# AlexeyAB/yolo2_light

Hardware: NVIDIA H100
Metric: images/sec (higher is better)
Workload: dtype bf16

## Files before the change

### yolo2_light_b200/csrc/yb_conv_tc.cu

```cuda
#include <cuda.h>
#include <cuda_bf16.h>
#include <cuda_runtime.h>

#include <algorithm>
#include <climits>
#include <cstdlib>
#include <cstring>
#include <memory>
#include <string>
#include <type_traits>
#include <vector>

#include "yb_conv_tc.cuh"
#include "yb_cuda.h"

namespace yb {

namespace {

constexpr int TC_BM = 128;
constexpr int TC_EPI_WARPS = 8;
constexpr int TC_THREADS = 32 * TC_EPI_WARPS + 32;
constexpr int TC_PRODUCER_WARP = TC_EPI_WARPS;
constexpr int TC_ACC_BAR = 3;

struct TcSmem {
    uint32_t ring;
    uint32_t full, empty;
    uint32_t bstat_bar;
    uint32_t stg_full, stg_ready;
    uint32_t bias;
    uint32_t ymask;
    uint32_t stg;
    uint32_t acc;
};

struct TcParams {
    int N;
    int TW, TWlog2, TH;
    int xt, jt, nt;
    int num_work;
    int kind;
    int kk;
    float alpha1;
    const float *mean;
    int xK;
    int *acc_out;
    float *yolo_out;
    int yolo_per;
    int PR, row_off;
    int OH, OW, OHp, OWp;
    int size, cblocks, kblocks;
    int BK, BN;
    int stride2;
    int xoff, yoff;
    int stages;
    uint32_t stage_bytes, a_bytes, b_bytes;
    int bstat;
    uint32_t bstat_bytes;
    int tma_epi;
    uint32_t stg_bytes;
    int acc_pitch;
    int pool_mode, jshift;
    float pool_mult;
    signed char *pool_out; long pool_ldc; int pool_Hp, pool_Wp;
    int sps;
    TcSmem sm;
    uint32_t desc_hi;
    char *out; long out_ldc; int n;
    const char *res;
    const float *bias; int act, act2;
    unsigned long long *stats;
    int dbg;
};

__device__ __forceinline__ uint32_t smem_u32(const void *p) { return (uint32_t)__cvta_generic_to_shared(p); }

__device__ __forceinline__ bool elect_one() {
    uint32_t pred = 0;
    asm volatile(
        "{\n\t.reg .b32 rx;\n\t.reg .pred px;\n\telect.sync rx|px, %1;\n\t@px mov.s32 %0, 1;\n\t}"
        : "+r"(pred) : "r"(0xffffffffu));
    return pred != 0;
}

__device__ __forceinline__ void mbar_init(uint32_t bar, uint32_t count) {
    asm volatile("mbarrier.init.shared::cta.b64 [%0], %1;" ::"r"(bar), "r"(count));
}
__device__ __forceinline__ void mbar_arrive_expect_tx(uint32_t bar, uint32_t bytes) {
    asm volatile("mbarrier.arrive.expect_tx.shared::cta.b64 _, [%0], %1;" ::"r"(bar), "r"(bytes) : "memory");
}
__device__ __forceinline__ void mbar_arrive(uint32_t bar) {
    asm volatile("mbarrier.arrive.shared::cta.b64 _, [%0];" ::"r"(bar) : "memory");
}
__device__ __forceinline__ uint32_t mbar_try_wait(uint32_t bar, uint32_t parity) {
    uint32_t ok;
    asm volatile(
        "{\n\t.reg .pred p;\n\tmbarrier.try_wait.parity.shared::cta.b64 p, [%1], %2;\n\tselp.b32 %0, 1, 0, p;\n\t}"
        : "=r"(ok) : "r"(bar), "r"(parity) : "memory");
    return ok;
}
__device__ __forceinline__ void mbar_wait(uint32_t bar, uint32_t parity) {
    if (mbar_try_wait(bar, parity)) return;
    const long long t0 = clock64();
    while (!mbar_try_wait(bar, parity))
        if (clock64() - t0 > 4000000000LL) __trap();
}

__device__ __forceinline__ void tma_load_3d(uint32_t dst, const CUtensorMap *tm, uint32_t bar, int c0, int c1, int c2) {
    asm volatile(
        "cp.async.bulk.tensor.3d.shared::cluster.global.tile.mbarrier::complete_tx::bytes [%0], [%1, {%3, %4, %5}], [%2];"
        ::"r"(dst), "l"(tm), "r"(bar), "r"(c0), "r"(c1), "r"(c2) : "memory");
}
__device__ __forceinline__ uint64_t l2_policy_evict_first() {
    uint64_t pol;
    asm volatile("createpolicy.fractional.L2::evict_first.b64 %0, 1.0;" : "=l"(pol));
    return pol;
}
__device__ __forceinline__ void tma_load_3d_hint(uint32_t dst, const CUtensorMap *tm, uint32_t bar, int c0, int c1, int c2, uint64_t pol) {
    asm volatile(
        "cp.async.bulk.tensor.3d.shared::cluster.global.tile.mbarrier::complete_tx::bytes.L2::cache_hint [%0], [%1, {%3, %4, %5}], [%2], %6;"
        ::"r"(dst), "l"(tm), "r"(bar), "r"(c0), "r"(c1), "r"(c2), "l"(pol) : "memory");
}
__device__ __forceinline__ void tma_load_2d(uint32_t dst, const CUtensorMap *tm, uint32_t bar, int c0, int c1) {
    asm volatile(
        "cp.async.bulk.tensor.2d.shared::cluster.global.tile.mbarrier::complete_tx::bytes [%0], [%1, {%3, %4}], [%2];"
        ::"r"(dst), "l"(tm), "r"(bar), "r"(c0), "r"(c1) : "memory");
}
__device__ __forceinline__ void tma_load_5d(uint32_t dst, const CUtensorMap *tm, uint32_t bar, int c0, int c1, int c2,
                                            int c3, int c4) {
    asm volatile(
        "cp.async.bulk.tensor.5d.shared::cluster.global.tile.mbarrier::complete_tx::bytes [%0], [%1, {%3, %4, %5, %6, %7}], [%2];"
        ::"r"(dst), "l"(tm), "r"(bar), "r"(c0), "r"(c1), "r"(c2), "r"(c3), "r"(c4) : "memory");
}

__device__ __forceinline__ void tma_store_3d(const CUtensorMap *tm, uint32_t src, int c0, int c1, int c2) {
    asm volatile("cp.async.bulk.tensor.3d.global.shared::cta.bulk_group [%0, {%2, %3, %4}], [%1];"
                 ::"l"(tm), "r"(src), "r"(c0), "r"(c1), "r"(c2) : "memory");
}
__device__ __forceinline__ void tma_store_commit() { asm volatile("cp.async.bulk.commit_group;" ::: "memory"); }
__device__ __forceinline__ void tma_store_wait_read0() { asm volatile("cp.async.bulk.wait_group.read 0;" ::: "memory"); }
__device__ __forceinline__ void tma_store_wait_all() { asm volatile("cp.async.bulk.wait_group 0;" ::: "memory"); }
__device__ __forceinline__ void named_bar_sync(int id, int nthreads) {
    asm volatile("bar.sync %0, %1;" ::"r"(id), "r"(nthreads) : "memory");
}
__device__ __forceinline__ void prefetch_tmap(const CUtensorMap *tm) { asm volatile("prefetch.tensormap [%0];" ::"l"(tm) : "memory"); }
__device__ __forceinline__ void fence_mbar_init() { asm volatile("fence.mbarrier_init.release.cluster;" ::: "memory"); }
__device__ __forceinline__ void pdl_wait_and_launch() {
    asm volatile("griddepcontrol.wait;" ::: "memory");
    asm volatile("griddepcontrol.launch_dependents;" ::: "memory");
}

__device__ __forceinline__ uint64_t wg_desc(uint32_t addr, uint32_t hi) {
    return ((uint64_t)hi << 32) | (uint64_t)(((addr & 0x3FFFFu) >> 4) | (1u << 16));
}
__device__ __forceinline__ void wg_fence() { asm volatile("wgmma.fence.sync.aligned;" ::: "memory"); }
__device__ __forceinline__ void wg_commit() { asm volatile("wgmma.commit_group.sync.aligned;" ::: "memory"); }
template <int N>
__device__ __forceinline__ void wg_wait() { asm volatile("wgmma.wait_group.sync.aligned %0;" ::"n"(N) : "memory"); }
template <typename T, int N>
__device__ __forceinline__ void wg_fence_operand(T (&d)[N]) {
#pragma unroll
    for (int i = 0; i < N; ++i) {
        if constexpr (std::is_same<T, float>::value) asm volatile("" : "+f"(d[i])::"memory");
        else asm volatile("" : "+r"(d[i])::"memory");
    }
}

template <TcKind KIND, int N> struct Wg;
template <> struct Wg<TC_BF16, 32> {
    static __device__ __forceinline__ void mma(float (&d)[16], uint64_t a, uint64_t b, uint32_t scale_d) {
        asm volatile(
            "{\n\t.reg .pred p;\n\tsetp.ne.b32 p, %18, 0;\n\t"
            "wgmma.mma_async.sync.aligned.m64n32k16.f32.bf16.bf16 "
            "{%0, %1, %2, %3, %4, %5, %6, %7, %8, %9, %10, %11, %12, %13, %14, %15}, %16, %17, p, 1, 1, 0, 0;\n\t}"
            : "+f"(d[0]), "+f"(d[1]), "+f"(d[2]), "+f"(d[3]), "+f"(d[4]), "+f"(d[5]), "+f"(d[6]), "+f"(d[7]), "+f"(d[8]), "+f"(d[9]), "+f"(d[10]), "+f"(d[11]), "+f"(d[12]), "+f"(d[13]), "+f"(d[14]), "+f"(d[15])
            : "l"(a), "l"(b), "r"(scale_d) : "memory");
    }
};
template <> struct Wg<TC_BF16, 64> {
    static __device__ __forceinline__ void mma(float (&d)[32], uint64_t a, uint64_t b, uint32_t scale_d) {
        asm volatile(
            "{\n\t.reg .pred p;\n\tsetp.ne.b32 p, %34, 0;\n\t"
            "wgmma.mma_async.sync.aligned.m64n64k16.f32.bf16.bf16 "
            "{%0, %1, %2, %3, %4, %5, %6, %7, %8, %9, %10, %11, %12, %13, %14, %15, %16, %17, %18, %19, %20, %21, %22, %23, %24, %25, %26, %27, %28, %29, %30, %31}, %32, %33, p, 1, 1, 0, 0;\n\t}"
            : "+f"(d[0]), "+f"(d[1]), "+f"(d[2]), "+f"(d[3]), "+f"(d[4]), "+f"(d[5]), "+f"(d[6]), "+f"(d[7]), "+f"(d[8]), "+f"(d[9]), "+f"(d[10]), "+f"(d[11]), "+f"(d[12]), "+f"(d[13]), "+f"(d[14]), "+f"(d[15]), "+f"(d[16]), "+f"(d[17]), "+f"(d[18]), "+f"(d[19]), "+f"(d[20]), "+f"(d[21]), "+f"(d[22]), "+f"(d[23]), "+f"(d[24]), "+f"(d[25]), "+f"(d[26]), "+f"(d[27]), "+f"(d[28]), "+f"(d[29]), "+f"(d[30]), "+f"(d[31])
            : "l"(a), "l"(b), "r"(scale_d) : "memory");
    }
};
template <> struct Wg<TC_BF16, 128> {
    static __device__ __forceinline__ void mma(float (&d)[64], uint64_t a, uint64_t b, uint32_t scale_d) {
        asm volatile(
            "{\n\t.reg .pred p;\n\tsetp.ne.b32 p, %66, 0;\n\t"
            "wgmma.mma_async.sync.aligned.m64n128k16.f32.bf16.bf16 "
            "{%0, %1, %2, %3, %4, %5, %6, %7, %8, %9, %10, %11, %12, %13, %14, %15, %16, %17, %18, %19, %20, %21, %22, %23, %24, %25, %26, %27, %28, %29, %30, %31, %32, %33, %34, %35, %36, %37, %38, %39, %40, %41, %42, %43, %44, %45, %46, %47, %48, %49, %50, %51, %52, %53, %54, %55, %56, %57, %58, %59, %60, %61, %62, %63}, %64, %65, p, 1, 1, 0, 0;\n\t}"
            : "+f"(d[0]), "+f"(d[1]), "+f"(d[2]), "+f"(d[3]), "+f"(d[4]), "+f"(d[5]), "+f"(d[6]), "+f"(d[7]), "+f"(d[8]), "+f"(d[9]), "+f"(d[10]), "+f"(d[11]), "+f"(d[12]), "+f"(d[13]), "+f"(d[14]), "+f"(d[15]), "+f"(d[16]), "+f"(d[17]), "+f"(d[18]), "+f"(d[19]), "+f"(d[20]), "+f"(d[21]), "+f"(d[22]), "+f"(d[23]), "+f"(d[24]), "+f"(d[25]), "+f"(d[26]), "+f"(d[27]), "+f"(d[28]), "+f"(d[29]), "+f"(d[30]), "+f"(d[31]), "+f"(d[32]), "+f"(d[33]), "+f"(d[34]), "+f"(d[35]), "+f"(d[36]), "+f"(d[37]), "+f"(d[38]), "+f"(d[39]), "+f"(d[40]), "+f"(d[41]), "+f"(d[42]), "+f"(d[43]), "+f"(d[44]), "+f"(d[45]), "+f"(d[46]), "+f"(d[47]), "+f"(d[48]), "+f"(d[49]), "+f"(d[50]), "+f"(d[51]), "+f"(d[52]), "+f"(d[53]), "+f"(d[54]), "+f"(d[55]), "+f"(d[56]), "+f"(d[57]), "+f"(d[58]), "+f"(d[59]), "+f"(d[60]), "+f"(d[61]), "+f"(d[62]), "+f"(d[63])
            : "l"(a), "l"(b), "r"(scale_d) : "memory");
    }
};
template <> struct Wg<TC_BF16, 256> {
    static __device__ __forceinline__ void mma(float (&d)[128], uint64_t a, uint64_t b, uint32_t scale_d) {
        asm volatile(
            "{\n\t.reg .pred p;\n\tsetp.ne.b32 p, %130, 0;\n\t"
            "wgmma.mma_async.sync.aligned.m64n256k16.f32.bf16.bf16 "
            "{%0, %1, %2, %3, %4, %5, %6, %7, %8, %9, %10, %11, %12, %13, %14, %15, %16, %17, %18, %19, %20, %21, %22, %23, %24, %25, %26, %27, %28, %29, %30, %31, %32, %33, %34, %35, %36, %37, %38, %39, %40, %41, %42, %43, %44, %45, %46, %47, %48, %49, %50, %51, %52, %53, %54, %55, %56, %57, %58, %59, %60, %61, %62, %63, %64, %65, %66, %67, %68, %69, %70, %71, %72, %73, %74, %75, %76, %77, %78, %79, %80, %81, %82, %83, %84, %85, %86, %87, %88, %89, %90, %91, %92, %93, %94, %95, %96, %97, %98, %99, %100, %101, %102, %103, %104, %105, %106, %107, %108, %109, %110, %111, %112, %113, %114, %115, %116, %117, %118, %119, %120, %121, %122, %123, %124, %125, %126, %127}, %128, %129, p, 1, 1, 0, 0;\n\t}"
            : "+f"(d[0]), "+f"(d[1]), "+f"(d[2]), "+f"(d[3]), "+f"(d[4]), "+f"(d[5]), "+f"(d[6]), "+f"(d[7]), "+f"(d[8]), "+f"(d[9]), "+f"(d[10]), "+f"(d[11]), "+f"(d[12]), "+f"(d[13]), "+f"(d[14]), "+f"(d[15]), "+f"(d[16]), "+f"(d[17]), "+f"(d[18]), "+f"(d[19]), "+f"(d[20]), "+f"(d[21]), "+f"(d[22]), "+f"(d[23]), "+f"(d[24]), "+f"(d[25]), "+f"(d[26]), "+f"(d[27]), "+f"(d[28]), "+f"(d[29]), "+f"(d[30]), "+f"(d[31]), "+f"(d[32]), "+f"(d[33]), "+f"(d[34]), "+f"(d[35]), "+f"(d[36]), "+f"(d[37]), "+f"(d[38]), "+f"(d[39]), "+f"(d[40]), "+f"(d[41]), "+f"(d[42]), "+f"(d[43]), "+f"(d[44]), "+f"(d[45]), "+f"(d[46]), "+f"(d[47]), "+f"(d[48]), "+f"(d[49]), "+f"(d[50]), "+f"(d[51]), "+f"(d[52]), "+f"(d[53]), "+f"(d[54]), "+f"(d[55]), "+f"(d[56]), "+f"(d[57]), "+f"(d[58]), "+f"(d[59]), "+f"(d[60]), "+f"(d[61]), "+f"(d[62]), "+f"(d[63]), "+f"(d[64]), "+f"(d[65]), "+f"(d[66]), "+f"(d[67]), "+f"(d[68]), "+f"(d[69]), "+f"(d[70]), "+f"(d[71]), "+f"(d[72]), "+f"(d[73]), "+f"(d[74]), "+f"(d[75]), "+f"(d[76]), "+f"(d[77]), "+f"(d[78]), "+f"(d[79]), "+f"(d[80]), "+f"(d[81]), "+f"(d[82]), "+f"(d[83]), "+f"(d[84]), "+f"(d[85]), "+f"(d[86]), "+f"(d[87]), "+f"(d[88]), "+f"(d[89]), "+f"(d[90]), "+f"(d[91]), "+f"(d[92]), "+f"(d[93]), "+f"(d[94]), "+f"(d[95]), "+f"(d[96]), "+f"(d[97]), "+f"(d[98]), "+f"(d[99]), "+f"(d[100]), "+f"(d[101]), "+f"(d[102]), "+f"(d[103]), "+f"(d[104]), "+f"(d[105]), "+f"(d[106]), "+f"(d[107]), "+f"(d[108]), "+f"(d[109]), "+f"(d[110]), "+f"(d[111]), "+f"(d[112]), "+f"(d[113]), "+f"(d[114]), "+f"(d[115]), "+f"(d[116]), "+f"(d[117]), "+f"(d[118]), "+f"(d[119]), "+f"(d[120]), "+f"(d[121]), "+f"(d[122]), "+f"(d[123]), "+f"(d[124]), "+f"(d[125]), "+f"(d[126]), "+f"(d[127])
            : "l"(a), "l"(b), "r"(scale_d) : "memory");
    }
};
template <> struct Wg<TC_S8, 32> {
    static __device__ __forceinline__ void mma(uint32_t (&d)[16], uint64_t a, uint64_t b, uint32_t scale_d) {
        asm volatile(
            "{\n\t.reg .pred p;\n\tsetp.ne.b32 p, %18, 0;\n\t"
            "wgmma.mma_async.sync.aligned.m64n32k32.s32.s8.s8 "
            "{%0, %1, %2, %3, %4, %5, %6, %7, %8, %9, %10, %11, %12, %13, %14, %15}, %16, %17, p;\n\t}"
            : "+r"(d[0]), "+r"(d[1]), "+r"(d[2]), "+r"(d[3]), "+r"(d[4]), "+r"(d[5]), "+r"(d[6]), "+r"(d[7]), "+r"(d[8]), "+r"(d[9]), "+r"(d[10]), "+r"(d[11]), "+r"(d[12]), "+r"(d[13]), "+r"(d[14]), "+r"(d[15])
            : "l"(a), "l"(b), "r"(scale_d) : "memory");
    }
};
template <> struct Wg<TC_S8, 64> {
    static __device__ __forceinline__ void mma(uint32_t (&d)[32], uint64_t a, uint64_t b, uint32_t scale_d) {
        asm volatile(
            "{\n\t.reg .pred p;\n\tsetp.ne.b32 p, %34, 0;\n\t"
            "wgmma.mma_async.sync.aligned.m64n64k32.s32.s8.s8 "
            "{%0, %1, %2, %3, %4, %5, %6, %7, %8, %9, %10, %11, %12, %13, %14, %15, %16, %17, %18, %19, %20, %21, %22, %23, %24, %25, %26, %27, %28, %29, %30, %31}, %32, %33, p;\n\t}"
            : "+r"(d[0]), "+r"(d[1]), "+r"(d[2]), "+r"(d[3]), "+r"(d[4]), "+r"(d[5]), "+r"(d[6]), "+r"(d[7]), "+r"(d[8]), "+r"(d[9]), "+r"(d[10]), "+r"(d[11]), "+r"(d[12]), "+r"(d[13]), "+r"(d[14]), "+r"(d[15]), "+r"(d[16]), "+r"(d[17]), "+r"(d[18]), "+r"(d[19]), "+r"(d[20]), "+r"(d[21]), "+r"(d[22]), "+r"(d[23]), "+r"(d[24]), "+r"(d[25]), "+r"(d[26]), "+r"(d[27]), "+r"(d[28]), "+r"(d[29]), "+r"(d[30]), "+r"(d[31])
            : "l"(a), "l"(b), "r"(scale_d) : "memory");
    }
};
template <> struct Wg<TC_S8, 128> {
    static __device__ __forceinline__ void mma(uint32_t (&d)[64], uint64_t a, uint64_t b, uint32_t scale_d) {
        asm volatile(
            "{\n\t.reg .pred p;\n\tsetp.ne.b32 p, %66, 0;\n\t"
            "wgmma.mma_async.sync.aligned.m64n128k32.s32.s8.s8 "
            "{%0, %1, %2, %3, %4, %5, %6, %7, %8, %9, %10, %11, %12, %13, %14, %15, %16, %17, %18, %19, %20, %21, %22, %23, %24, %25, %26, %27, %28, %29, %30, %31, %32, %33, %34, %35, %36, %37, %38, %39, %40, %41, %42, %43, %44, %45, %46, %47, %48, %49, %50, %51, %52, %53, %54, %55, %56, %57, %58, %59, %60, %61, %62, %63}, %64, %65, p;\n\t}"
            : "+r"(d[0]), "+r"(d[1]), "+r"(d[2]), "+r"(d[3]), "+r"(d[4]), "+r"(d[5]), "+r"(d[6]), "+r"(d[7]), "+r"(d[8]), "+r"(d[9]), "+r"(d[10]), "+r"(d[11]), "+r"(d[12]), "+r"(d[13]), "+r"(d[14]), "+r"(d[15]), "+r"(d[16]), "+r"(d[17]), "+r"(d[18]), "+r"(d[19]), "+r"(d[20]), "+r"(d[21]), "+r"(d[22]), "+r"(d[23]), "+r"(d[24]), "+r"(d[25]), "+r"(d[26]), "+r"(d[27]), "+r"(d[28]), "+r"(d[29]), "+r"(d[30]), "+r"(d[31]), "+r"(d[32]), "+r"(d[33]), "+r"(d[34]), "+r"(d[35]), "+r"(d[36]), "+r"(d[37]), "+r"(d[38]), "+r"(d[39]), "+r"(d[40]), "+r"(d[41]), "+r"(d[42]), "+r"(d[43]), "+r"(d[44]), "+r"(d[45]), "+r"(d[46]), "+r"(d[47]), "+r"(d[48]), "+r"(d[49]), "+r"(d[50]), "+r"(d[51]), "+r"(d[52]), "+r"(d[53]), "+r"(d[54]), "+r"(d[55]), "+r"(d[56]), "+r"(d[57]), "+r"(d[58]), "+r"(d[59]), "+r"(d[60]), "+r"(d[61]), "+r"(d[62]), "+r"(d[63])
            : "l"(a), "l"(b), "r"(scale_d) : "memory");
    }
};
template <> struct Wg<TC_TF32, 32> {
    static __device__ __forceinline__ void mma(float (&d)[16], uint64_t a, uint64_t b, uint32_t scale_d) {
        asm volatile(
            "{\n\t.reg .pred p;\n\tsetp.ne.b32 p, %18, 0;\n\t"
            "wgmma.mma_async.sync.aligned.m64n32k8.f32.tf32.tf32 "
            "{%0, %1, %2, %3, %4, %5, %6, %7, %8, %9, %10, %11, %12, %13, %14, %15}, %16, %17, p, 1, 1;\n\t}"
            : "+f"(d[0]), "+f"(d[1]), "+f"(d[2]), "+f"(d[3]), "+f"(d[4]), "+f"(d[5]), "+f"(d[6]), "+f"(d[7]), "+f"(d[8]), "+f"(d[9]), "+f"(d[10]), "+f"(d[11]), "+f"(d[12]), "+f"(d[13]), "+f"(d[14]), "+f"(d[15])
            : "l"(a), "l"(b), "r"(scale_d) : "memory");
    }
};
template <> struct Wg<TC_TF32, 64> {
    static __device__ __forceinline__ void mma(float (&d)[32], uint64_t a, uint64_t b, uint32_t scale_d) {
        asm volatile(
            "{\n\t.reg .pred p;\n\tsetp.ne.b32 p, %34, 0;\n\t"
            "wgmma.mma_async.sync.aligned.m64n64k8.f32.tf32.tf32 "
            "{%0, %1, %2, %3, %4, %5, %6, %7, %8, %9, %10, %11, %12, %13, %14, %15, %16, %17, %18, %19, %20, %21, %22, %23, %24, %25, %26, %27, %28, %29, %30, %31}, %32, %33, p, 1, 1;\n\t}"
            : "+f"(d[0]), "+f"(d[1]), "+f"(d[2]), "+f"(d[3]), "+f"(d[4]), "+f"(d[5]), "+f"(d[6]), "+f"(d[7]), "+f"(d[8]), "+f"(d[9]), "+f"(d[10]), "+f"(d[11]), "+f"(d[12]), "+f"(d[13]), "+f"(d[14]), "+f"(d[15]), "+f"(d[16]), "+f"(d[17]), "+f"(d[18]), "+f"(d[19]), "+f"(d[20]), "+f"(d[21]), "+f"(d[22]), "+f"(d[23]), "+f"(d[24]), "+f"(d[25]), "+f"(d[26]), "+f"(d[27]), "+f"(d[28]), "+f"(d[29]), "+f"(d[30]), "+f"(d[31])
            : "l"(a), "l"(b), "r"(scale_d) : "memory");
    }
};
template <> struct Wg<TC_TF32, 128> {
    static __device__ __forceinline__ void mma(float (&d)[64], uint64_t a, uint64_t b, uint32_t scale_d) {
        asm volatile(
            "{\n\t.reg .pred p;\n\tsetp.ne.b32 p, %66, 0;\n\t"
            "wgmma.mma_async.sync.aligned.m64n128k8.f32.tf32.tf32 "
            "{%0, %1, %2, %3, %4, %5, %6, %7, %8, %9, %10, %11, %12, %13, %14, %15, %16, %17, %18, %19, %20, %21, %22, %23, %24, %25, %26, %27, %28, %29, %30, %31, %32, %33, %34, %35, %36, %37, %38, %39, %40, %41, %42, %43, %44, %45, %46, %47, %48, %49, %50, %51, %52, %53, %54, %55, %56, %57, %58, %59, %60, %61, %62, %63}, %64, %65, p, 1, 1;\n\t}"
            : "+f"(d[0]), "+f"(d[1]), "+f"(d[2]), "+f"(d[3]), "+f"(d[4]), "+f"(d[5]), "+f"(d[6]), "+f"(d[7]), "+f"(d[8]), "+f"(d[9]), "+f"(d[10]), "+f"(d[11]), "+f"(d[12]), "+f"(d[13]), "+f"(d[14]), "+f"(d[15]), "+f"(d[16]), "+f"(d[17]), "+f"(d[18]), "+f"(d[19]), "+f"(d[20]), "+f"(d[21]), "+f"(d[22]), "+f"(d[23]), "+f"(d[24]), "+f"(d[25]), "+f"(d[26]), "+f"(d[27]), "+f"(d[28]), "+f"(d[29]), "+f"(d[30]), "+f"(d[31]), "+f"(d[32]), "+f"(d[33]), "+f"(d[34]), "+f"(d[35]), "+f"(d[36]), "+f"(d[37]), "+f"(d[38]), "+f"(d[39]), "+f"(d[40]), "+f"(d[41]), "+f"(d[42]), "+f"(d[43]), "+f"(d[44]), "+f"(d[45]), "+f"(d[46]), "+f"(d[47]), "+f"(d[48]), "+f"(d[49]), "+f"(d[50]), "+f"(d[51]), "+f"(d[52]), "+f"(d[53]), "+f"(d[54]), "+f"(d[55]), "+f"(d[56]), "+f"(d[57]), "+f"(d[58]), "+f"(d[59]), "+f"(d[60]), "+f"(d[61]), "+f"(d[62]), "+f"(d[63])
            : "l"(a), "l"(b), "r"(scale_d) : "memory");
    }
};
template <int N> struct Wg<TC_XNOR, N> : Wg<TC_S8, N> {};

__device__ __forceinline__ uint32_t pack_bf16x2(float a, float b) {
    __nv_bfloat162 h = __floats2bfloat162_rn(a, b);
    return *reinterpret_cast<uint32_t *>(&h);
}

__device__ __forceinline__ void acc_ld32(uint32_t addr, uint32_t (&v)[32]) {
#pragma unroll
    for (int c = 0; c < 8; ++c)
        asm volatile("ld.shared.v4.b32 {%0, %1, %2, %3}, [%4];" : "=r"(v[4 * c]), "=r"(v[4 * c + 1]), "=r"(v[4 * c + 2]), "=r"(v[4 * c + 3])
                     : "r"(addr + 16u * (uint32_t)c) : "memory");
}
template <typename T, int NR>
__device__ __forceinline__ void acc_store_frag(uint32_t acc, int pitch, int row0, const T (&d)[NR]) {
    const int lane = threadIdx.x & 31, w = (threadIdx.x >> 5) & 3;
    const int r = row0 + 16 * w + (lane >> 2), c = 2 * (lane & 3);
    const uint32_t a0 = acc + 4u * (uint32_t)(r * pitch + c), a1 = a0 + 4u * 8u * (uint32_t)pitch;
#pragma unroll
    for (int j = 0; j < NR / 4; ++j) {
        asm volatile("st.shared.v2.b32 [%0], {%1, %2};" ::"r"(a0 + 32u * (uint32_t)j), "r"(*reinterpret_cast<const uint32_t *>(&d[4 * j])),
                     "r"(*reinterpret_cast<const uint32_t *>(&d[4 * j + 1])) : "memory");
        asm volatile("st.shared.v2.b32 [%0], {%1, %2};" ::"r"(a1 + 32u * (uint32_t)j), "r"(*reinterpret_cast<const uint32_t *>(&d[4 * j + 2])),
                     "r"(*reinterpret_cast<const uint32_t *>(&d[4 * j + 3])) : "memory");
    }
}

__device__ __forceinline__ uint32_t smem_base(const void *smem_raw) { return (smem_u32(smem_raw) + 1023u) & ~1023u; }
__device__ __forceinline__ void *smem_ptr(uint32_t addr) { return __cvta_shared_to_generic(addr); }
__device__ __forceinline__ void st_shared_u32(uint32_t addr, uint32_t v) {
    asm volatile("st.shared.b32 [%0], %1;" ::"r"(addr), "r"(v) : "memory");
}

struct TcItem { int n0, x0, J0; };
__device__ __forceinline__ TcItem tc_item(const TcParams &p, int w, int BN) {
    const int m = w / p.nt;
    return {(w % p.nt) * BN, (m % p.xt) * p.TW, (m / p.xt) * p.TH + p.jshift};
}
struct TcPixel {
    int img, oy, ox;
    __device__ __forceinline__ bool valid(const TcParams &p) const { return img < p.N && oy >= 0 && oy < p.OH && ox < p.OW; }
};
__device__ __forceinline__ TcPixel tc_pixel(const TcParams &p, const TcItem &t, int r) {
    const int J = t.J0 + (r >> p.TWlog2);
    const int img = J / p.PR;
    return {img, J - img * p.PR - p.row_off, t.x0 + (r & (p.TW - 1))};
}

struct TcRing {
    int stage = 0;
    uint32_t phase = 0;
    __device__ __forceinline__ void advance(int stages) { if (++stage == stages) { stage = 0; phase ^= 1u; } }
};
__device__ __forceinline__ void tc_init_ring(const TcParams &p, uint32_t base) {
    for (int s = 0; s < p.stages; ++s) { mbar_init(base + p.sm.full + 8u * s, 1); mbar_init(base + p.sm.empty + 8u * s, TC_EPI_WARPS); }
    mbar_init(base + p.sm.bstat_bar, 1);
}

template <int BN_MAX, typename F>
__device__ __forceinline__ void tc_dispatch(const TcParams &p, F &&f) {
    auto by_kk = [&](auto bn_c) {
        if (p.kk == 4) f(bn_c, std::integral_constant<int, 4>{});
        else if (p.kk == 2) f(bn_c, std::integral_constant<int, 2>{});
        else f(bn_c, std::integral_constant<int, 1>{});
    };
    if constexpr (BN_MAX == 256) {
        if (p.BN == 256) { by_kk(std::integral_constant<int, 256>{}); return; }
    }
    if (p.BN == 128) by_kk(std::integral_constant<int, 128>{});
    else if (p.BN == 64) by_kk(std::integral_constant<int, 64>{});
    else by_kk(std::integral_constant<int, 32>{});
}

enum TcStat {
    STAT_PROD_WAIT_EMPTY,
    STAT_PROD_TMA_ISSUE,
    STAT_PROD_TOTAL,
    STAT_CONS_WAIT_FULL,
    STAT_CONS_WAIT_READY,
    STAT_CONS_FIRST_READY,
    STAT_CONS_TOTAL,
    STAT_STORE_WAIT_FULL,
    STAT_STORE_WAIT_READ,
    TC_NSTATS = 16
};
__device__ __forceinline__ unsigned long long &tc_stat(const TcParams &p, TcStat s) { return p.stats[blockIdx.x * TC_NSTATS + s]; }
template <bool ST, typename F>
__device__ __forceinline__ void timed(long long &cycles, F &&f) {
    if constexpr (ST) { const long long c0 = clock64(); f(); cycles += clock64() - c0; }
    else f();
}

template <bool ST>
__device__ __forceinline__ void tc_produce(const CUtensorMap *tmA, const CUtensorMap *tmB, const TcParams &p, uint32_t base,
                                           int w_first, int w_step) {
    TcRing ring;
    long long w_empty = 0, w_tma = 0; const long long t_begin = ST ? clock64() : 0;
    const int sps = p.sps, kblocks = p.kblocks, cblocks = p.cblocks, BK = p.BK, fsize = p.size, stages = p.stages;
    const int xoff = p.xoff, yoff = p.yoff, stride2 = p.stride2;
    const uint32_t a_bytes = p.a_bytes, b_bytes = p.b_bytes, stage_bytes = p.stage_bytes;
    const uint32_t b_off = (uint32_t)sps * a_bytes;
    const uint32_t smemB = base, smem0 = base + p.sm.ring, bstat_bar = base + p.sm.bstat_bar;
    const int bstat = p.bstat;
    if (bstat) {
        mbar_arrive_expect_tx(bstat_bar, p.bstat_bytes);
        for (int kb = 0; kb < kblocks; ++kb) tma_load_2d(smemB + (uint32_t)kb * b_bytes, tmB, bstat_bar, kb * BK, 0);
    }
    for (int w = w_first; w < p.num_work; w += w_step) {
        const TcItem it = tc_item(p, w, p.BN);
        int cb = 0, ky = 0, kx = 0, kcol = 0;
        for (int kb0 = 0; kb0 < kblocks; kb0 += sps) {
            const int nsub = min(sps, kblocks - kb0);
            timed<ST>(w_empty, [&] { mbar_wait(base + p.sm.empty + 8u * (uint32_t)ring.stage, ring.phase ^ 1u); });
            const uint32_t fb = base + p.sm.full + 8u * (uint32_t)ring.stage;
            const uint32_t a_dst = smem0 + (uint32_t)ring.stage * stage_bytes;
            const uint32_t b_dst = a_dst + b_off;
            if (p.dbg & 1) {
                mbar_arrive(fb);
                ring.advance(stages);
                continue;
            }
            mbar_arrive_expect_tx(fb, (uint32_t)nsub * (a_bytes + (bstat ? 0u : b_bytes)));
            timed<ST>(w_tma, [&] {
                for (int j = 0; j < nsub; ++j) {
                    const uint32_t ad = a_dst + (uint32_t)j * a_bytes, bd = b_dst + (uint32_t)j * b_bytes;
                    const int c0 = cb * BK;
                    if (stride2) tma_load_5d(ad, tmA, fb, c0, kx & 1, it.x0 + (kx >> 1), ky & 1, it.J0 + (ky >> 1));
                    else tma_load_3d(ad, tmA, fb, c0, it.x0 + kx + xoff, it.J0 + ky + yoff);
                    if (!bstat) tma_load_2d(bd, tmB, fb, kcol, it.n0);
                    kcol += BK;
                    if (++cb == cblocks) { cb = 0; if (++kx == fsize) { kx = 0; ++ky; } }
                }
            });
            ring.advance(stages);
        }
    }
    if (ST && p.stats) {
        tc_stat(p, STAT_PROD_WAIT_EMPTY) = w_empty; tc_stat(p, STAT_PROD_TMA_ISSUE) = w_tma;
        tc_stat(p, STAT_PROD_TOTAL) = clock64() - t_begin;
    }
}

template <TcKind KIND, int BN, int KK, bool ST, typename T>
__device__ __forceinline__ void tc_mma_loop(T (&d)[BN / 2], const TcParams &p, uint32_t base, int wg, int lane, TcRing &ring,
                                            long long &w_full) {
#pragma unroll
    for (int i = 0; i < BN / 2; ++i) d[i] = T(0);
    wg_fence_operand(d);
    const int sps = p.sps, stages = p.stages, kblocks = p.kblocks;
    const uint32_t a_bytes = p.a_bytes, b_bytes = p.b_bytes, stage_bytes = p.stage_bytes, hi = p.desc_hi;
    const uint32_t b_off = (uint32_t)sps * a_bytes, a_wg = (uint32_t)wg * (a_bytes >> 1);
    const uint32_t smemB = base, smem0 = base + p.sm.ring;
    const uint32_t full = base + p.sm.full, empty = base + p.sm.empty;
    auto release = [&](int s) { __syncwarp(); if (lane == 0) mbar_arrive(empty + 8u * (uint32_t)s); };
    int pend = -1, jj = 0;
    for (int kb = 0; kb < kblocks; ++kb) {
        if (jj == 0) timed<ST>(w_full, [&] { mbar_wait(full + 8u * (uint32_t)ring.stage, ring.phase); });
        const uint32_t st_base = smem0 + (uint32_t)ring.stage * stage_bytes;
        const uint32_t a_kb = st_base + a_wg + (uint32_t)jj * a_bytes;
        const uint32_t b_kb = p.bstat ? smemB + (uint32_t)kb * b_bytes : st_base + b_off + (uint32_t)jj * b_bytes;
        wg_fence();
#pragma unroll
        for (int k = 0; k < KK; ++k)
            Wg<KIND, BN>::mma(d, wg_desc(a_kb + 32u * (uint32_t)k, hi), wg_desc(b_kb + 32u * (uint32_t)k, hi),
                              (kb > 0 || k > 0) ? 1u : 0u);
        wg_commit();
        wg_wait<1>();
        if (pend >= 0) { release(pend); pend = -1; }
        if (++jj == sps || kb + 1 == kblocks) {
            pend = ring.stage; jj = 0;
            ring.advance(stages);
        }
    }
    wg_wait<0>();
    wg_fence_operand(d);
    if (pend >= 0) release(pend);
}

__device__ __forceinline__ float int_epilogue(const TcParams &p, int kind, int acc, int f, float bias) {
    if (kind == TC_S8) {
        int q16 = acc / 32;
        q16 = q16 > 32767 ? 32767 : (q16 < -32767 ? -32767 : q16);
        const float t = __fadd_rn(__fmul_rn((float)q16, p.alpha1), bias);
        return (p.act == ACT_LEAKY) ? ((t > 0.f) ? t : __fdiv_rn(t, 10.f)) : t;
    }
    const float t = __fadd_rn(__fmul_rn((float)acc, (f < p.n) ? __ldg(p.mean + f) : 0.f), bias);
    return act_exact(t, p.act);
}

template <bool ST, int EPI>
__global__ void __launch_bounds__(TC_THREADS, 1)
k_conv_tc(const __grid_constant__ CUtensorMap tmA, const __grid_constant__ CUtensorMap tmB, const __grid_constant__ CUtensorMap tmO,
          const __grid_constant__ CUtensorMap tmO1, const __grid_constant__ CUtensorMap tmR, const TcParams p) {
    extern __shared__ uint8_t smem_raw[];
    const uint32_t base = smem_base(smem_raw);

    const int warp = __shfl_sync(0xffffffffu, (int)(threadIdx.x >> 5), 0);
    const int lane = threadIdx.x & 31;
    const int w_first = (int)blockIdx.x, w_step = (int)gridDim.x;

    if (warp == TC_PRODUCER_WARP && elect_one()) {
        prefetch_tmap(&tmA);
        prefetch_tmap(&tmB);
        tc_init_ring(p, base);
        if (p.tma_epi) prefetch_tmap(&tmO);
        fence_mbar_init();
    }
    const float *bias_s = reinterpret_cast<const float *>(smem_ptr(base + p.sm.bias));
    const uint32_t *ymask_s = reinterpret_cast<const uint32_t *>(smem_ptr(base + p.sm.ymask));
    const uint32_t stg_base = base + p.sm.stg;
    const uint32_t acc_base = base + p.sm.acc;
    for (int i = threadIdx.x; i < p.nt * p.BN; i += TC_THREADS)
        st_shared_u32(base + p.sm.bias + 4u * (uint32_t)i, __float_as_uint((i < p.n) ? __ldg(p.bias + i) : 0.f));
    if (p.yolo_out) {
        for (int wd = threadIdx.x; wd < p.nt * p.BN / 32; wd += TC_THREADS) {
            uint32_t m = 0;
            for (int j = 0; j < 32; ++j) { const int e = (wd * 32 + j) % p.yolo_per; if (e == 2 || e == 3) m |= 1u << j; }
            st_shared_u32(base + p.sm.ymask + 4u * (uint32_t)wd, m);
        }
    }
    __syncthreads();
    pdl_wait_and_launch();

    if (warp == TC_PRODUCER_WARP) {
        if (elect_one()) tc_produce<ST>(&tmA, &tmB, p, base, w_first, w_step);
    } else {
        const int ew = warp;
        const int wg = ew >> 2;
        TcRing ring;
        long long w_full = 0;
        if (p.bstat) mbar_wait(base + p.sm.bstat_bar, 0);
        auto mainloop = [&](auto kind_c) {
            tc_dispatch<128>(p, [&](auto bn_c, auto kk_c) {
                constexpr TcKind KIND = decltype(kind_c)::value;
                constexpr int BN = decltype(bn_c)::value;
                constexpr int KK = decltype(kk_c)::value;
                using T = typename std::conditional<KIND == TC_S8 || KIND == TC_XNOR, uint32_t, float>::type;
                T d[BN / 2];
                tc_mma_loop<KIND, BN, KK, ST>(d, p, base, wg, lane, ring, w_full);
                named_bar_sync(TC_ACC_BAR, 32 * TC_EPI_WARPS);
                acc_store_frag(acc_base, p.acc_pitch, wg * 64, d);
                named_bar_sync(TC_ACC_BAR, 32 * TC_EPI_WARPS);
            });
        };
        auto run_mainloop = [&]() {
            if constexpr (EPI == 2) mainloop(std::integral_constant<TcKind, TC_S8>{});
            else if (p.kind == TC_BF16) mainloop(std::integral_constant<TcKind, TC_BF16>{});
            else mainloop(std::integral_constant<TcKind, TC_TF32>{});
        };

        const int q = ew & 3;
        const int half = ew >> 2;
        const int cbeg = (p.BN >= 64) ? half * (p.BN >> 1) : 0;
        const int cend = (p.BN >= 64) ? cbeg + (p.BN >> 1) : (half == 0 ? p.BN : 0);
        const int r = q * 32 + lane;
        const bool leaky = p.act == ACT_LEAKY;
        const uint32_t taddr = acc_base + 4u * (uint32_t)(r * p.acc_pitch);
        const long long t_begin = ST ? clock64() : 0;
        for (int w = w_first; w < p.num_work; w += w_step) {
            run_mainloop();
            const TcItem it = tc_item(p, w, p.BN);
            const TcPixel px = tc_pixel(p, it, r);
            const int n0 = it.n0, img = px.img, oy = px.oy, ox = px.ox;
            const bool valid = px.valid(p) && !(p.dbg & 4);
            const long pix = ((long)(img * p.OHp + oy + 1) * p.OWp + ox + 1);
            char *orow = p.out + pix * p.out_ldc * 4;
            const float *bs = bias_s + n0;

            auto finish_f32 = [&](const uint32_t (&v)[32], int f0) {
                if (!valid || (n0 + f0) >= p.n) return;
                float x[32];
#pragma unroll
                for (int j = 0; j < 32; ++j) {
                    float a = __uint_as_float(v[j]) + bs[f0 + j];
                    x[j] = leaky ? fmaxf(a, 0.1f * a) : a;
                }
                if (p.yolo_out) {
                    const int c0 = n0 + f0;
                    const int nvalid = p.n - c0;
                    const uint32_t raw = ymask_s[c0 >> 5];
                    float *dst = p.yolo_out + (((size_t)img * p.n + c0) * p.OH + oy) * (size_t)p.OW + ox;
                    const size_t plane = (size_t)p.OH * p.OW;
#pragma unroll
                    for (int j = 0; j < 32; ++j) {
                        const float sg = __fdividef(1.f, 1.f + __expf(-x[j]));
                        const float v = ((raw >> j) & 1u) ? x[j] : sg;
                        if (j < nvalid) dst[(size_t)j * plane] = v;
                    }
                } else {
                    float4 *op = reinterpret_cast<float4 *>(orow + (size_t)(n0 + f0) * 4);
#pragma unroll
                    for (int g = 0; g < 8; ++g) {
                        const int left = p.n - (n0 + f0 + g * 4);
                        if (left <= 0) break;
                        if (left >= 4) op[g] = make_float4(x[g * 4 + 0], x[g * 4 + 1], x[g * 4 + 2], x[g * 4 + 3]);
                        else {
#pragma unroll
                            for (int e = 0; e < 3; ++e)
                                if (e < left) reinterpret_cast<float *>(op + g)[e] = x[g * 4 + e];
                        }
                    }
                }
            };

            auto store_f32_slab = [&](const float (&y)[32], int f0) {
                const uint32_t stg = stg_base + (uint32_t)ew * 4096u;
                const int srow = lane >> 3, schunk = lane & 7;
                const unsigned long long obase = (unsigned long long)(uintptr_t)orow;
                const int vflag = valid ? 1 : 0;
#pragma unroll
                for (int c = 0; c < 8; ++c)
                    asm volatile("st.shared.v4.b32 [%0], {%1, %2, %3, %4};" ::"r"(stg + (uint32_t)lane * 128u + (uint32_t)((c ^ (lane & 7)) << 4)),
                                 "r"(__float_as_uint(y[c * 4 + 0])), "r"(__float_as_uint(y[c * 4 + 1])),
                                 "r"(__float_as_uint(y[c * 4 + 2])), "r"(__float_as_uint(y[c * 4 + 3])) : "memory");
                __syncwarp();
#pragma unroll
                for (int i = 0; i < 8; ++i) {
                    const int row = i * 4 + srow;
                    const unsigned long long op = __shfl_sync(0xffffffffu, obase, row);
                    const int ok = __shfl_sync(0xffffffffu, vflag, row);
                    uint32_t w0, w1, w2, w3;
                    asm volatile("ld.shared.v4.b32 {%0, %1, %2, %3}, [%4];" : "=r"(w0), "=r"(w1), "=r"(w2), "=r"(w3)
                                 : "r"(stg + (uint32_t)row * 128u + (uint32_t)((schunk ^ (row & 7)) << 4)) : "memory");
                    const int left = p.n - (n0 + f0 + schunk * 4);
                    uint4 *dst = reinterpret_cast<uint4 *>(op + (size_t)(n0 + f0) * 4) + schunk;
                    if (ok && left >= 4) *dst = make_uint4(w0, w1, w2, w3);
                    else if (ok && left > 0) {
                        uint32_t *d1 = reinterpret_cast<uint32_t *>(dst);
                        d1[0] = w0;
                        if (left > 1) d1[1] = w1;
                        if (left > 2) d1[2] = w2;
                    }
                }
                __syncwarp();
            };

            auto pool_store_raw = [&](const uint32_t (&v)[32], int f0) {
                const bool b0 = lane & 1, b3 = lane & 8;
                int h16[16], h8[8];
#pragma unroll
                for (int j = 0; j < 16; ++j) {
                    const int lo_ = valid ? (int)v[j] : INT_MIN, hi_ = valid ? (int)v[j + 16] : INT_MIN;
                    const int keep = b0 ? hi_ : lo_, send = b0 ? lo_ : hi_;
                    const int got = __shfl_xor_sync(0xffffffffu, send, 1);
                    h16[j] = max(keep, got);
                }
#pragma unroll
                for (int j = 0; j < 8; ++j) {
                    const int keep = b3 ? h16[j + 8] : h16[j], send = b3 ? h16[j] : h16[j + 8];
                    const int got = __shfl_xor_sync(0xffffffffu, send, 8);
                    h8[j] = max(keep, got);
                }
                const int cbase = f0 + (b0 ? 16 : 0) + (b3 ? 8 : 0);
                uint32_t w0 = 0, w1 = 0;
#pragma unroll
                for (int j = 0; j < 8; ++j) {
                    const int f = n0 + cbase + j;
                    const float t = int_epilogue(p, p.kind, h8[j], f, bs[cbase + j]);
                    int b8 = (p.pool_mode == 1) ? quant_i8(t, p.pool_mult) : (t > 0.f ? 1 : -1);
                    if (f >= p.n) b8 = 0;
                    if (j < 4) w0 |= (uint32_t)(b8 & 0xff) << (8 * j); else w1 |= (uint32_t)(b8 & 0xff) << (8 * (j - 4));
                }
                const TcPixel o{img, oy & ~1, ox & ~1};
                if (o.valid(p) && !(p.dbg & 4)) {
                    signed char *dst = p.pool_out + ((size_t)(img * p.pool_Hp + (o.oy >> 1) + 1) * p.pool_Wp + (o.ox >> 1) + 1) * (size_t)p.pool_ldc + n0 + cbase;
                    *reinterpret_cast<uint2 *>(dst) = make_uint2(w0, w1);
                }
            };

            auto tma_store_f32_slab = [&](const float (&y)[32], int f0) {
                const int g = half;
                const uint32_t out_tile = stg_base + (uint32_t)g * 16384u;
                const bool boss = (q == 0) && (lane == 0);
                const uint32_t rsw = (uint32_t)(r & 7), row_off = (uint32_t)r * 128u;
                if (boss) tma_store_wait_read0();
                named_bar_sync(1 + g, 128);
#pragma unroll
                for (int c = 0; c < 8; ++c) {
                    uint32_t o0 = __float_as_uint(y[c * 4 + 0]), o1 = __float_as_uint(y[c * 4 + 1]);
                    uint32_t o2 = __float_as_uint(y[c * 4 + 2]), o3 = __float_as_uint(y[c * 4 + 3]);
                    if (!valid) { o0 = o1 = o2 = o3 = 0u; }
                    asm volatile("st.shared.v4.b32 [%0], {%1, %2, %3, %4};" ::"r"(out_tile + row_off + (((uint32_t)c ^ rsw) << 4)),
                                 "r"(o0), "r"(o1), "r"(o2), "r"(o3) : "memory");
                }
                asm volatile("fence.proxy.async.shared::cta;" ::: "memory");
                named_bar_sync(1 + g, 128);
                if (boss) {
                    const TcItem t = tc_item(p, w, p.BN);
                    tma_store_3d(&tmO, out_tile, n0 + f0, t.x0 + 1, t.J0);
                    tma_store_commit();
                }
            };

            if constexpr (EPI == 2) {
                auto int_slabs = [&](auto kind_c) {
                    constexpr TcKind KIND = decltype(kind_c)::value;
                    for (int f0 = cbeg; f0 < cend; f0 += 32) {
                        uint32_t v0[32];
                        acc_ld32(taddr + 4u * (uint32_t)f0, v0);
                        if (p.pool_mode) { pool_store_raw(v0, f0); continue; }
                        float y[32];
#pragma unroll
                        for (int j = 0; j < 32; ++j) y[j] = int_epilogue(p, KIND, (int)v0[j], n0 + f0 + j, bs[f0 + j]);
                        if (p.tma_epi) tma_store_f32_slab(y, f0);
                        else store_f32_slab(y, f0);
                        if (!valid || !p.acc_out) continue;
#pragma unroll
                        for (int j = 0; j < 32; ++j) {
                            const int f = n0 + f0 + j;
                            if (f < p.n) p.acc_out[(((size_t)img * p.n + f) * p.OH + oy) * p.OW + ox] = KIND == TC_XNOR ? ((int)v0[j] + p.xK) / 2 : (int)v0[j];
                        }
                    }
                };
                if (p.kind == TC_XNOR) int_slabs(std::integral_constant<TcKind, TC_XNOR>{});
                else int_slabs(std::integral_constant<TcKind, TC_S8>{});
            } else {
                for (int f0 = cbeg; f0 < cend; f0 += 64) {
                    if (cend - f0 >= 64) {
                        uint32_t v0[32], v1[32];
                        acc_ld32(taddr + 4u * (uint32_t)f0, v0);
                        acc_ld32(taddr + 4u * (uint32_t)f0 + 128u, v1);
                        finish_f32(v0, f0);
                        finish_f32(v1, f0 + 32);
                    } else {
                        uint32_t v0[32];
                        acc_ld32(taddr + 4u * (uint32_t)f0, v0);
                        finish_f32(v0, f0);
                    }
                }
            }
        }
        if (EPI == 2 && p.tma_epi && q == 0 && lane == 0) tma_store_wait_all();
        if (ST && p.stats && ew == 0 && lane == 0) { tc_stat(p, STAT_CONS_WAIT_FULL) = w_full; tc_stat(p, STAT_CONS_TOTAL) = clock64() - t_begin; }
    }
}

constexpr int TCR_THREADS = 384;
constexpr int TCR_PRODUCER_REGS = 40, TCR_CONSUMER_REGS = 216;
constexpr int TCR_STORE_WARP = 9;
constexpr int TCR_MAX_SLABS = 4;

template <bool ST>
__device__ __forceinline__ void tcr_store(const CUtensorMap *tmO, const CUtensorMap *tmO1, const CUtensorMap *tmR, const TcParams &p,
                                          uint32_t buf, uint32_t stg_full, uint32_t stg_ready, int g, int w_first, int w_step) {
    const int SW = p.tma_epi, BN = p.BN;
    const uint32_t tile = 64u * 2u * (uint32_t)SW;
    const int hx = (p.TW == 128) ? 64 * g : 0, hy = (p.TW == 128) ? 0 : g * (p.TH >> 1);
    long long w_full = 0, w_read = 0;
    auto item = [&](int w, int &n0, int &x, int &y) {
        const TcItem it = tc_item(p, w, BN);
        n0 = it.n0; x = it.x0 + 1 + hx; y = it.J0 + hy;
        if (p.stride2) {
            const int i0 = y / p.PR, i1 = min((y + max(p.TH >> 1, 1) - 1) / p.PR, p.N - 1);
            y = i0 == i1 ? y + i0 + 1 : -1 - y;
        }
        return (min(BN, p.n - n0) + SW - 1) / SW;
    };
    auto store_slab = [&](uint32_t src, int c, int x, int y) {
        if (y >= 0) { tma_store_3d(tmO, src, c, x, y); return; }
        const int J0 = -1 - y;
        int img = J0 / p.PR, oy = J0 - img * p.PR;
        for (int t = 0; t < (p.TH >> 1); ++t) {
            if (img < p.N && oy < p.OH) tma_store_3d(tmO1, src, c, x, J0 + t + img + 1);
            if (++oy == p.PR) { oy = 0; ++img; }
            src += (uint32_t)(p.TW * 2 * SW);
        }
    };
    auto wait_read = [&]() { timed<ST>(w_read, tma_store_wait_read0); };
    auto load_res = [&](int s, int n0, int x, int y) {
        tma_load_3d_hint(buf + (uint32_t)s * tile, tmR, stg_ready, n0 + s * SW, x, y, l2_policy_evict_first());
    };
    if (w_first < p.num_work) {
        if (p.res) {
            int n0, x, y;
            const int ns = item(w_first, n0, x, y);
            mbar_arrive_expect_tx(stg_ready, (uint32_t)ns * tile);
            for (int s = 0; s < ns; ++s) load_res(s, n0, x, y);
        } else mbar_arrive(stg_ready);
    }
    uint32_t phases = 0;
    for (int w = w_first; w < p.num_work; w += w_step) {
        int n0, x, y, n0n = 0, xn = 0, yn = 0;
        const int ns = item(w, n0, x, y);
        const bool next = w + w_step < p.num_work, res_next = next && p.res;
        const int nsn = next ? item(w + w_step, n0n, xn, yn) : 0;
        for (int s = 0; s < ns; ++s) {
            const uint32_t fb = stg_full + 8u * (uint32_t)s;
            timed<ST>(w_full, [&] { mbar_wait(fb, (phases >> s) & 1u); });
            phases ^= 1u << s;
            if (s == 0 && res_next) mbar_arrive_expect_tx(stg_ready, (uint32_t)nsn * tile);
            store_slab(buf + (uint32_t)s * tile, n0 + s * SW, x, y);
            tma_store_commit();
            if (res_next && s < nsn) { wait_read(); load_res(s, n0n, xn, yn); }
        }
        if (res_next) {
            for (int s = ns; s < nsn; ++s) { wait_read(); load_res(s, n0n, xn, yn); }
        } else if (next) {
            wait_read();
            mbar_arrive(stg_ready);
        }
    }
    tma_store_wait_all();
    if (ST && p.stats && g == 0) { tc_stat(p, STAT_STORE_WAIT_FULL) = w_full; tc_stat(p, STAT_STORE_WAIT_READ) = w_read; }
}

template <bool ST>
__global__ void __launch_bounds__(TCR_THREADS, 1)
k_conv_tc_reg(const __grid_constant__ CUtensorMap tmA, const __grid_constant__ CUtensorMap tmB, const __grid_constant__ CUtensorMap tmO,
              const __grid_constant__ CUtensorMap tmO1, const __grid_constant__ CUtensorMap tmR, const TcParams p) {
    extern __shared__ uint8_t smem_raw[];
    const uint32_t base = smem_base(smem_raw);
    auto stg_full = [&](int g, int s) { return base + p.sm.stg_full + 8u * (uint32_t)(g * TCR_MAX_SLABS + s); };
    auto stg_ready = [&](int g) { return base + p.sm.stg_ready + 8u * (uint32_t)g; };
    float *bias_s = reinterpret_cast<float *>(smem_ptr(base + p.sm.bias));
    const uint32_t stg_base = base + p.sm.stg;

    const int warp = __shfl_sync(0xffffffffu, (int)(threadIdx.x >> 5), 0);
    const int lane = threadIdx.x & 31;
    const int wg = warp >> 2;
    const int w_first = (int)blockIdx.x, w_step = (int)gridDim.x;
    const bool epi_mem = !(p.dbg & 4);

    if (warp == TC_PRODUCER_WARP && elect_one()) {
        prefetch_tmap(&tmA);
        prefetch_tmap(&tmB);
        prefetch_tmap(&tmO);
        if (p.stride2) prefetch_tmap(&tmO1);
        if (p.res) prefetch_tmap(&tmR);
        tc_init_ring(p, base);
        for (int g = 0; g < 2; ++g) {
            for (int s = 0; s < TCR_MAX_SLABS; ++s) mbar_init(stg_full(g, s), 4);
            mbar_init(stg_ready(g), 1);
        }
        fence_mbar_init();
    }
    for (int i = threadIdx.x; i < p.nt * p.BN; i += TCR_THREADS) bias_s[i] = (i < p.n) ? __ldg(p.bias + i) : 0.f;
    __syncthreads();
    pdl_wait_and_launch();

    if (wg == 2) {
        asm volatile("setmaxnreg.dec.sync.aligned.u32 %0;" ::"n"(TCR_PRODUCER_REGS));
        if (warp == TC_PRODUCER_WARP) {
            if (elect_one()) tc_produce<ST>(&tmA, &tmB, p, base, w_first, w_step);
        } else if (warp < TCR_STORE_WARP + 2 && epi_mem) {
            const int g = warp - TCR_STORE_WARP;
            if (elect_one()) tcr_store<ST>(&tmO, &tmO1, &tmR, p, stg_base + (uint32_t)g * 128u * (uint32_t)p.BN, stg_full(g, 0), stg_ready(g), g, w_first, w_step);
        }
        return;
    }
    asm volatile("setmaxnreg.inc.sync.aligned.u32 %0;" ::"n"(TCR_CONSUMER_REGS));

    const int rl = 16 * (warp & 3) + (lane >> 2), cq = 2 * (lane & 3);
    const bool leaky = p.act == ACT_LEAKY, leaky2 = p.act2 == ACT_LEAKY;
    const bool has_res = p.res != nullptr;
    TcRing ring;
    uint32_t stg_phase = 0;
    long long w_full = 0, w_ready = 0; const long long t_begin = ST ? clock64() : 0;
    if (p.bstat) mbar_wait(base + p.sm.bstat_bar, 0);

    tc_dispatch<256>(p, [&](auto bn_c, auto kk_c) {
        constexpr int BN = decltype(bn_c)::value;
        constexpr int KK = decltype(kk_c)::value;
        constexpr int SW = BN >= 64 ? 64 : 32;
        constexpr uint32_t ROWB = SW * 2, TILE = 64u * ROWB;
        const uint32_t buf = stg_base + (uint32_t)wg * (uint32_t)(BN / SW) * TILE;
        auto slab_off = [&](int row, int c) -> uint32_t {
            const int sw = (SW == 64) ? (row & 7) : ((row >> 1) & 3);
            return (uint32_t)row * ROWB + ((uint32_t)(c ^ sw) << 4) + 2u * (uint32_t)cq;
        };
        for (int w = w_first; w < p.num_work; w += w_step) {
            float d[BN / 2];
            tc_mma_loop<TC_BF16, BN, KK, ST>(d, p, base, wg, lane, ring, w_full);
            if (!epi_mem) continue;
            const TcItem it = tc_item(p, w, BN);
            const int n0 = it.n0;
            bool valid[2];
#pragma unroll
            for (int h = 0; h < 2; ++h)
                valid[h] = tc_pixel(p, it, 64 * wg + rl + 8 * h).valid(p);
            const int nslab = (min(BN, p.n - n0) + SW - 1) / SW;
            long long dt = 0;
            timed<ST>(dt, [&] { mbar_wait(stg_ready(wg), stg_phase); });
            if (w != w_first) w_ready += dt;
            else if (ST && p.stats && warp == 0 && lane == 0) tc_stat(p, STAT_CONS_FIRST_READY) = dt;
            stg_phase ^= 1u;
#pragma unroll
            for (int s = 0; s < BN / SW; ++s) {
                if (s >= nslab) break;
                const uint32_t slab = buf + (uint32_t)s * TILE;
#pragma unroll
                for (int jj = 0; jj < SW / 8; ++jj) {
                    const int j = s * (SW / 8) + jj;
                    const float2 b = *reinterpret_cast<const float2 *>(bias_s + n0 + 8 * j + cq);
#pragma unroll
                    for (int e = 0; e < 4; ++e) {
                        const float a = d[4 * j + e] + ((e & 1) ? b.y : b.x);
                        d[4 * j + e] = leaky ? fmaxf(a, 0.1f * a) : a;
                    }
                }
                if (has_res) {
                    uint32_t u[SW / 8][2];
#pragma unroll
                    for (int jj = 0; jj < SW / 8; ++jj)
#pragma unroll
                        for (int h = 0; h < 2; ++h)
                            asm volatile("ld.shared.b32 %0, [%1];" : "=r"(u[jj][h]) : "r"(slab + slab_off(rl + 8 * h, jj)));
#pragma unroll
                    for (int jj = 0; jj < SW / 8; ++jj) {
                        const int j = s * (SW / 8) + jj;
#pragma unroll
                        for (int h = 0; h < 2; ++h) {
                            float a = d[4 * j + 2 * h] + __uint_as_float(u[jj][h] << 16);
                            float c = d[4 * j + 2 * h + 1] + __uint_as_float(u[jj][h] & 0xffff0000u);
                            if (leaky2) { a = fmaxf(a, 0.1f * a); c = fmaxf(c, 0.1f * c); }
                            d[4 * j + 2 * h] = a; d[4 * j + 2 * h + 1] = c;
                        }
                    }
                }
#pragma unroll
                for (int jj = 0; jj < SW / 8; ++jj) {
                    const int j = s * (SW / 8) + jj;
#pragma unroll
                    for (int h = 0; h < 2; ++h) {
                        const uint32_t o = valid[h] ? pack_bf16x2(d[4 * j + 2 * h], d[4 * j + 2 * h + 1]) : 0u;
                        asm volatile("st.shared.b32 [%0], %1;" ::"r"(slab + slab_off(rl + 8 * h, jj)), "r"(o));
                    }
                }
                asm volatile("fence.proxy.async.shared::cta;" ::: "memory");
                __syncwarp();
                if (lane == 0) mbar_arrive(stg_full(wg, s));
            }
        }
    });
    if (ST && p.stats && warp == 0 && lane == 0) {
        tc_stat(p, STAT_CONS_WAIT_FULL) = w_full; tc_stat(p, STAT_CONS_WAIT_READY) = w_ready;
        tc_stat(p, STAT_CONS_TOTAL) = clock64() - t_begin;
    }
}

struct StemTcP {
    const float *in;
    const unsigned char *in8;
    char *out; int out_ldc;
    const __nv_bfloat16 *w;
    const float *bias;
    int N, H, W, OHp, OWp, nf, act;
    long npix;
    int ntiles;
    const __nv_bfloat16 *w1;
    const float *bias1;
    int act1, OH, OW, xt, yt;
};

template <bool U8>
__global__ void __launch_bounds__(128) k_stem_tc(StemTcP p) {
    __shared__ __align__(1024) uint8_t a_tile[128 * 64];
    __shared__ __align__(1024) uint8_t b_tile[32 * 64];
    __shared__ __align__(16) float acc_s[128 * 36];
    __shared__ float bias_s[32];
    __shared__ unsigned long long optr[128];
    __shared__ float lut[U8 ? 256 : 1];
    const int t = threadIdx.x;
    if constexpr (U8) { lut[t] = (float)((double)(float)t / 255.0); lut[t + 128] = (float)((double)(float)(t + 128) / 255.0); }
    const uint32_t a_addr = smem_u32(a_tile), b_addr = smem_u32(b_tile), acc_addr = smem_u32(acc_s);
    if (t < 32) bias_s[t] = (t < p.nf) ? p.bias[t] : 0.f;
    {
        const int f = t >> 2, j = t & 3;
        const uint4 v = *reinterpret_cast<const uint4 *>(p.w + f * 32 + j * 8);
        *reinterpret_cast<uint4 *>(b_tile + f * 64 + ((j ^ ((f >> 1) & 3)) << 4)) = v;
    }
    __syncthreads();
    const uint32_t hi = ((8u * 64u) >> 4) | (2u << 30);
    const size_t plane = (size_t)p.H * p.W;
    for (int tile = blockIdx.x; tile < p.ntiles; tile += gridDim.x) {
        const unsigned pix = (unsigned)tile * 128u + (unsigned)t;
        const bool ok = pix < (unsigned)p.npix;
        int x = 0, y = 0, n = 0;
        if (ok) { const unsigned row = pix / (unsigned)p.W; x = (int)(pix - row * (unsigned)p.W); n = (int)(row / (unsigned)p.H); y = (int)(row - (unsigned)n * (unsigned)p.H); }
        uint32_t packed[16];
        {
            float v[32];
            if constexpr (U8) {
                const unsigned char *img8 = p.in8 + (size_t)n * 3 * plane;
                if (ok && x >= 1 && x + 1 < p.W && y >= 1 && y + 1 < p.H) {
                    const unsigned char *r1 = img8 + ((size_t)y * p.W + x) * 3, *r0 = r1 - (size_t)p.W * 3, *r2 = r1 + (size_t)p.W * 3;
#pragma unroll
                    for (int j = 0; j < 9; ++j) {
                        v[0 * 9 + j] = lut[__ldg(r0 - 3 + j)];
                        v[1 * 9 + j] = lut[__ldg(r1 - 3 + j)];
                        v[2 * 9 + j] = lut[__ldg(r2 - 3 + j)];
                    }
                } else {
#pragma unroll
                    for (int ky = 0; ky < 3; ++ky)
#pragma unroll
                        for (int kx = 0; kx < 3; ++kx) {
                            const int iy = y + ky - 1, ix = x + kx - 1;
                            const bool in_img = ok && iy >= 0 && iy < p.H && ix >= 0 && ix < p.W;
#pragma unroll
                            for (int c = 0; c < 3; ++c)
                                v[(ky * 3 + kx) * 3 + c] = in_img ? lut[__ldg(img8 + ((size_t)iy * p.W + ix) * 3 + c)] : 0.f;
                        }
                }
            } else {
            const float *img = p.in + (size_t)n * 3 * plane;
            if (ok && x >= 1 && x + 1 < p.W && y >= 1 && y + 1 < p.H) {
                const float *c0 = img + (size_t)y * p.W + x;
#pragma unroll
                for (int c = 0; c < 3; ++c) {
                    const float *r1 = c0 + (size_t)c * plane, *r0 = r1 - p.W, *r2 = r1 + p.W;
                    v[(0 * 3 + 0) * 3 + c] = __ldg(r0 - 1); v[(0 * 3 + 1) * 3 + c] = __ldg(r0); v[(0 * 3 + 2) * 3 + c] = __ldg(r0 + 1);
                    v[(1 * 3 + 0) * 3 + c] = __ldg(r1 - 1); v[(1 * 3 + 1) * 3 + c] = __ldg(r1); v[(1 * 3 + 2) * 3 + c] = __ldg(r1 + 1);
                    v[(2 * 3 + 0) * 3 + c] = __ldg(r2 - 1); v[(2 * 3 + 1) * 3 + c] = __ldg(r2); v[(2 * 3 + 2) * 3 + c] = __ldg(r2 + 1);
                }
            } else {
#pragma unroll
            for (int ky = 0; ky < 3; ++ky)
#pragma unroll
                for (int kx = 0; kx < 3; ++kx) {
                    const int iy = y + ky - 1, ix = x + kx - 1;
                    const bool in_img = ok && iy >= 0 && iy < p.H && ix >= 0 && ix < p.W;
#pragma unroll
                    for (int c = 0; c < 3; ++c)
                        v[(ky * 3 + kx) * 3 + c] = in_img ? __ldg(img + (size_t)c * plane + (size_t)iy * p.W + ix) : 0.f;
                }
            }
            }
#pragma unroll
            for (int k = 27; k < 32; ++k) v[k] = 0.f;
#pragma unroll
            for (int k = 0; k < 16; ++k) packed[k] = pack_bf16x2(v[2 * k], v[2 * k + 1]);
        }
#pragma unroll
        for (int j = 0; j < 4; ++j)
            *reinterpret_cast<uint4 *>(a_tile + t * 64 + ((j ^ ((t >> 1) & 3)) << 4)) =
                make_uint4(packed[4 * j], packed[4 * j + 1], packed[4 * j + 2], packed[4 * j + 3]);
        asm volatile("fence.proxy.async.shared::cta;" ::: "memory");
        __syncthreads();
        {
            float d0[16], d1[16];
#pragma unroll
            for (int i = 0; i < 16; ++i) { d0[i] = 0.f; d1[i] = 0.f; }
            wg_fence();
#pragma unroll
            for (int k = 0; k < 2; ++k) {
                const uint64_t bdesc = wg_desc(b_addr + 32u * k, hi);
                Wg<TC_BF16, 32>::mma(d0, wg_desc(a_addr + 32u * k, hi), bdesc, (uint32_t)k);
                Wg<TC_BF16, 32>::mma(d1, wg_desc(a_addr + 64u * 64u + 32u * k, hi), bdesc, (uint32_t)k);
            }
            wg_commit();
            wg_wait<0>();
            acc_store_frag(acc_addr, 36, 0, d0);
            acc_store_frag(acc_addr, 36, 64, d1);
        }
        __syncthreads();
        uint32_t acc[32];
        acc_ld32(acc_addr + 4u * 36u * (uint32_t)t, acc);
        char *orow = ok ? p.out + ((size_t)(n * p.OHp + y + 1) * p.OWp + x + 1) * (size_t)p.out_ldc * 2 : nullptr;
        if (p.nf == 32) {
            uint4 o[4];
#pragma unroll
            for (int g = 0; g < 4; ++g) {
                float r[8];
#pragma unroll
                for (int j = 0; j < 8; ++j) {
                    const float a = __uint_as_float(acc[g * 8 + j]) + bias_s[g * 8 + j];
                    r[j] = (p.act == ACT_LEAKY) ? fmaxf(a, 0.1f * a) : a;
                }
                o[g] = make_uint4(pack_bf16x2(r[0], r[1]), pack_bf16x2(r[2], r[3]), pack_bf16x2(r[4], r[5]), pack_bf16x2(r[6], r[7]));
            }
#pragma unroll
            for (int g = 0; g < 4; ++g) *reinterpret_cast<uint4 *>(a_tile + t * 64 + ((g ^ ((t >> 1) & 3)) << 4)) = o[g];
            optr[t] = (unsigned long long)(uintptr_t)orow;
            __syncthreads();
#pragma unroll
            for (int k = 0; k < 4; ++k) {
                const int j = t + 128 * k, px = j >> 2, part = j & 3;
                const unsigned long long dst = optr[px];
                if (dst)
                    *reinterpret_cast<uint4 *>(dst + (unsigned long long)(part * 16)) =
                        *reinterpret_cast<const uint4 *>(a_tile + px * 64 + ((part ^ ((px >> 1) & 3)) << 4));
            }
        } else if (ok) {
#pragma unroll
            for (int g = 0; g < 4; ++g) {
                if (g * 8 >= p.nf) break;
                float r[8];
#pragma unroll
                for (int j = 0; j < 8; ++j) {
                    const float a = __uint_as_float(acc[g * 8 + j]) + bias_s[g * 8 + j];
                    r[j] = (p.act == ACT_LEAKY) ? fmaxf(a, 0.1f * a) : a;
                }
                reinterpret_cast<uint4 *>(orow)[g] = make_uint4(pack_bf16x2(r[0], r[1]), pack_bf16x2(r[2], r[3]),
                                                                pack_bf16x2(r[4], r[5]), pack_bf16x2(r[6], r[7]));
            }
        }
        __syncthreads();
    }
}

constexpr int S2_TW = 16, S2_TH = 8;
constexpr int S2_RW = 2 * S2_TW + 1, S2_RH = 2 * S2_TH + 1;
constexpr int S2_ROWS = 640;
constexpr uint32_t S2_B1 = 0;
constexpr uint32_t S2_BS = 9u * 4096u;
constexpr uint32_t S2_U = S2_BS + 2048u;
constexpr uint32_t S2_SETS_KX = 17u * 1024u;
constexpr uint32_t S2_STG = (uint32_t)S2_ROWS * 64u;
constexpr uint32_t S2_MISC = S2_U + S2_STG + 2u * 8192u;
constexpr int S2_PH = S2_RH + 2, S2_PW = S2_RW + 2, S2_PP = 36;
constexpr size_t S2_SMEM = 1024 + S2_MISC + 4 * (32 + 64 + 256) + 4 * 3 * S2_PH * S2_PP;
static_assert(S2_STG + 2u * 8192u >= 3u * S2_SETS_KX, "sets must fit the shared region");

template <bool U8>
__global__ void __launch_bounds__(256, 2) k_stem_s2_tc(StemTcP p) {
    extern __shared__ uint8_t smem_raw[];
    uint8_t *sm = smem_raw + ((1024u - (smem_u32(smem_raw) & 1023u)) & 1023u);
    const uint32_t base = smem_u32(sm), U = base + S2_U;
    float *bias0_s = reinterpret_cast<float *>(sm + S2_MISC), *bias1_s = bias0_s + 32, *lut = bias1_s + 64, *patch = lut + 256;
    const int t = threadIdx.x, lane = t & 31;
    const int warp = __shfl_sync(0xffffffffu, t >> 5, 0), wg = warp >> 2;
    if constexpr (U8) lut[t] = (float)((double)(float)t / 255.0);
    if (t < 32) bias0_s[t] = p.bias[t];
    if (t < 64) bias1_s[t] = p.bias1[t];
    if (t < 128) {
        const int f = t >> 2, j = t & 3;
        *reinterpret_cast<uint4 *>(sm + S2_BS + f * 64 + ((j ^ ((f >> 1) & 3)) << 4)) = *reinterpret_cast<const uint4 *>(p.w + f * 32 + j * 8);
    }
    for (int i = t; i < 9 * 64 * 4; i += 256) {
        const int r = i >> 8, f = (i >> 2) & 63, j = i & 3;
        *reinterpret_cast<uint4 *>(sm + S2_B1 + r * 4096 + f * 64 + ((j ^ ((f >> 1) & 3)) << 4)) =
            *reinterpret_cast<const uint4 *>(p.w1 + f * 288 + r * 32 + j * 8);
    }
    asm volatile("fence.proxy.async.shared::cta;" ::: "memory");
    __syncthreads();

    const uint32_t hi = ((8u * 64u) >> 4) | (2u << 30);
    const bool leaky0 = p.act == ACT_LEAKY, leaky1 = p.act1 == ACT_LEAKY;
    const int rl = 16 * (warp & 3) + (lane >> 2), cq = 2 * (lane & 3);
    constexpr int PER = (3 * S2_PH * S2_PW + 255) / 256;
    auto patch_index = [&](int e, int &c, int &r, int &col) {
        if constexpr (U8) { r = e / (3 * S2_PW); const int b = e - r * 3 * S2_PW; col = b / 3; c = b - col * 3; }
        else { c = e / (S2_PH * S2_PW); const int b = e - c * S2_PH * S2_PW; r = b / S2_PW; col = b - r * S2_PW; }
    };
    auto load_patch = [&](int tile, float (&v)[PER]) {
        const int tx = tile % p.xt, rest = tile / p.xt, ty = rest % p.yt, n = rest / p.yt;
        const int py0 = 2 * ty * S2_TH - 2, px0 = 2 * tx * S2_TW - 2;
        const size_t img = (size_t)n * 3 * p.H * p.W;
#pragma unroll
        for (int k = 0; k < PER; ++k) {
            const int e = t + 256 * k;
            int c, r, col;
            patch_index(e, c, r, col);
            const int y = py0 + r, x = px0 + col;
            const bool in_img = e < 3 * S2_PH * S2_PW && y >= 0 && y < p.H && x >= 0 && x < p.W;
            if constexpr (U8) v[k] = in_img ? lut[__ldg(p.in8 + img + (unsigned)((y * p.W + x) * 3 + c))] : 0.f;
            else v[k] = in_img ? __ldg(p.in + img + (unsigned)((c * p.H + y) * p.W + x)) : 0.f;
        }
    };
    float pv[PER];
    if ((int)blockIdx.x < p.ntiles) load_patch(blockIdx.x, pv);
    for (int tile = blockIdx.x; tile < p.ntiles; tile += gridDim.x) {
        const int tx = tile % p.xt, rest = tile / p.xt, ty = rest % p.yt, n = rest / p.yt;
        const int ox0 = tx * S2_TW, oy0 = ty * S2_TH;
        const int gy0 = 2 * oy0 - 1, gx0 = 2 * ox0 - 1;

#pragma unroll
        for (int k = 0; k < PER; ++k) {
            const int e = t + 256 * k;
            if (e >= 3 * S2_PH * S2_PW) break;
            int c, r, col;
            patch_index(e, c, r, col);
            patch[(c * S2_PH + r) * S2_PP + col] = pv[k];
        }
        __syncthreads();

        for (int i = t; i < S2_ROWS; i += 256) {
            const int sy = i / S2_RW, sx = i - sy * S2_RW;
            const float *w0 = patch + sy * S2_PP + sx;
            const bool ok = i < S2_RW * S2_RH;
            uint32_t packed[16];
            {
                float v[32];
#pragma unroll
                for (int ky = 0; ky < 3; ++ky)
#pragma unroll
                    for (int kx = 0; kx < 3; ++kx)
#pragma unroll
                        for (int c = 0; c < 3; ++c) v[(ky * 3 + kx) * 3 + c] = ok ? w0[(c * S2_PH + ky) * S2_PP + kx] : 0.f;
#pragma unroll
                for (int k = 27; k < 32; ++k) v[k] = 0.f;
#pragma unroll
                for (int k = 0; k < 16; ++k) packed[k] = pack_bf16x2(v[2 * k], v[2 * k + 1]);
            }
#pragma unroll
            for (int j = 0; j < 4; ++j)
                *reinterpret_cast<uint4 *>(sm + S2_U + i * 64 + ((j ^ ((i >> 1) & 3)) << 4)) =
                    make_uint4(packed[4 * j], packed[4 * j + 1], packed[4 * j + 2], packed[4 * j + 3]);
        }
        asm volatile("fence.proxy.async.shared::cta;" ::: "memory");
        __syncthreads();

        float ds[5][16];
#pragma unroll
        for (int c = 0; c < 5; ++c)
#pragma unroll
            for (int i = 0; i < 16; ++i) ds[c][i] = 0.f;
#pragma unroll
        for (int c = 0; c < 5; ++c) wg_fence_operand(ds[c]);
        wg_fence();
#pragma unroll
        for (int c = 0; c < 5; ++c)
#pragma unroll
            for (int k = 0; k < 2; ++k)
                Wg<TC_BF16, 32>::mma(ds[c], wg_desc(U + (uint32_t)(5 * wg + c) * 4096u + 32u * k, hi), wg_desc(base + S2_BS + 32u * k, hi), (uint32_t)k);
        wg_commit();
        wg_wait<0>();
#pragma unroll
        for (int c = 0; c < 5; ++c) wg_fence_operand(ds[c]);
        __syncthreads();

        {
#pragma unroll
            for (int c = 0; c < 5; ++c)
#pragma unroll
                for (int h = 0; h < 2; ++h) {
                    const int i = 64 * (5 * wg + c) + rl + 8 * h;
                    if (i >= S2_RW * S2_RH) continue;
                    const int sy = i / S2_RW, sx = i - sy * S2_RW, y = gy0 + sy, x = gx0 + sx;
                    const bool in_img = y >= 0 && y < p.H && x >= 0 && x < p.W;
                    uint32_t v[4];
#pragma unroll
                    for (int j = 0; j < 4; ++j) {
                        float a = ds[c][4 * j + 2 * h] + bias0_s[8 * j + cq], b = ds[c][4 * j + 2 * h + 1] + bias0_s[8 * j + cq + 1];
                        if (leaky0) { a = fmaxf(a, 0.1f * a); b = fmaxf(b, 0.1f * b); }
                        v[j] = in_img ? pack_bf16x2(a, b) : 0u;
                    }
                    const uint32_t set = U + ((sy & 1) ? 9u * 1024u : 0u) + (uint32_t)(sy >> 1) * 1024u + 2u * (uint32_t)cq;
                    auto put = [&](int kx, int ox) {
                        const uint32_t row = set + (uint32_t)kx * S2_SETS_KX + (uint32_t)ox * 64u;
#pragma unroll
                        for (int j = 0; j < 4; ++j)
                            asm volatile("st.shared.b32 [%0], %1;" ::"r"(row + ((uint32_t)(j ^ ((ox >> 1) & 3)) << 4)), "r"(v[j]));
                    };
                    const bool odd = sx & 1, last = sx == 2 * S2_TW;
                    put(odd ? 1 : last ? 2 : 0, last ? (sx >> 1) - 1 : sx >> 1);
                    if (!odd && !last && sx >= 2) put(2, (sx >> 1) - 1);
                }
        }
        asm volatile("fence.proxy.async.shared::cta;" ::: "memory");
        __syncthreads();

        if (tile + (int)gridDim.x < p.ntiles) load_patch(tile + gridDim.x, pv);

        float d[32];
#pragma unroll
        for (int i = 0; i < 32; ++i) d[i] = 0.f;
        wg_fence_operand(d);
        wg_fence();
#pragma unroll
        for (int r = 0; r < 9; ++r) {
            const int ky = r / 3, kx = r % 3;
            const uint32_t a = U + (uint32_t)kx * S2_SETS_KX + ((ky & 1) ? 9u * 1024u : 0u) + (uint32_t)(ky >> 1) * 1024u + (uint32_t)wg * 4096u;
            const uint32_t b = base + S2_B1 + (uint32_t)r * 4096u;
#pragma unroll
            for (int k = 0; k < 2; ++k)
                Wg<TC_BF16, 64>::mma(d, wg_desc(a + 32u * k, hi), wg_desc(b + 32u * k, hi), (r > 0 || k > 0) ? 1u : 0u);
        }
        wg_commit();
        wg_wait<0>();
        wg_fence_operand(d);
        __syncthreads();

        const uint32_t stg = U + S2_STG + (uint32_t)wg * 8192u;
        float b1[16];
#pragma unroll
        for (int j = 0; j < 8; ++j) { b1[2 * j] = bias1_s[8 * j + cq]; b1[2 * j + 1] = bias1_s[8 * j + cq + 1]; }
#pragma unroll
        for (int h = 0; h < 2; ++h) {
            const int q = rl + 8 * h;
#pragma unroll
            for (int j = 0; j < 8; ++j) {
                float a = d[4 * j + 2 * h] + b1[2 * j], b = d[4 * j + 2 * h + 1] + b1[2 * j + 1];
                if (leaky1) { a = fmaxf(a, 0.1f * a); b = fmaxf(b, 0.1f * b); }
                asm volatile("st.shared.b32 [%0], %1;" ::"r"(stg + (uint32_t)q * 128u + ((uint32_t)(j ^ (q & 7)) << 4) + 2u * (uint32_t)cq),
                             "r"(pack_bf16x2(a, b)) : "memory");
            }
        }
        if (wg == 0) named_bar_sync(1, 128);
        else named_bar_sync(2, 128);
#pragma unroll
        for (int k = 0; k < 4; ++k) {
            const int idx = (t & 127) + 128 * k, q = idx >> 3, ch = idx & 7;
            const int oy = oy0 + 4 * wg + (q >> 4), ox = ox0 + (q & 15);
            if (oy < p.OH && ox < p.OW) {
                uint4 o;
                asm volatile("ld.shared.v4.b32 {%0, %1, %2, %3}, [%4];" : "=r"(o.x), "=r"(o.y), "=r"(o.z), "=r"(o.w)
                             : "r"(stg + (uint32_t)q * 128u + ((uint32_t)(ch ^ (q & 7)) << 4)) : "memory");
                *reinterpret_cast<uint4 *>(p.out + ((size_t)(n * p.OHp + oy + 1) * p.OWp + ox + 1) * (size_t)p.out_ldc * 2 + ch * 16) = o;
            }
        }
    }
}

typedef CUresult (*EncodeTiledFn)(CUtensorMap *, CUtensorMapDataType, cuuint32_t, void *, const cuuint64_t *,
                                  const cuuint64_t *, const cuuint32_t *, const cuuint32_t *, CUtensorMapInterleave,
                                  CUtensorMapSwizzle, CUtensorMapL2promotion, CUtensorMapFloatOOBfill);

EncodeTiledFn encode_fn() {
    static EncodeTiledFn fn = nullptr;
    if (!fn) {
        void *p = nullptr;
        cudaDriverEntryPointQueryResult q;
        if (cudaGetDriverEntryPoint("cuTensorMapEncodeTiled", &p, cudaEnableDefault, &q) != cudaSuccess || !p)
            fatal_throw("cuTensorMapEncodeTiled not available from the driver");
        fn = reinterpret_cast<EncodeTiledFn>(p);
    }
    return fn;
}

}

using TcKernel = void (*)(CUtensorMap, CUtensorMap, CUtensorMap, CUtensorMap, CUtensorMap, TcParams);

struct TcPlan {
    CUtensorMap tmA, tmB, tmO, tmO1, tmR;
    TcParams p;
    TcKernel kernel;
    bool reg;
    int grid;
    size_t smem;
    char desc[96];
    DevBuf<unsigned long long> stats;
};

namespace {

int sm_count() {
    int dev = 0, sms = 132;
    cudaGetDevice(&dev);
    cudaDeviceGetAttribute(&sms, cudaDevAttrMultiProcessorCount, dev);
    return sms;
}

bool is_integer(int kind) { return kind == TC_S8 || kind == TC_XNOR; }
int elem_size(int kind) { return kind == TC_TF32 ? 4 : is_integer(kind) ? 1 : 2; }
int operand_channels(const TcConv &c) { return is_integer(c.kind) ? c.in.ldc : c.l->c; }

bool geometry_ok(const Layer &l) {
    if (l.stride == 1) return (l.size == 3 && l.pad == 1) || (l.size == 1 && l.pad == 0);
    return l.stride == 2 && l.size == 3 && l.pad == 1 && l.h % 2 == 0 && l.w % 2 == 0;
}

int channel_row(int channels, int esz) {
    for (int bytes = 128; bytes >= 32; bytes /= 2)
        if (channels * esz % bytes == 0) return bytes / esz;
    return 0;
}

int pick_bn(int n) { return n <= 32 ? 32 : n <= 64 ? 64 : 128; }
int pick_bn_reg(int n, long m_tiles, int kblocks, int sms, int forced) {
    int cap = 32;
    while (cap < n && cap < 256) cap *= 2;
    if (forced > 0) {
        int bn = 32;
        while (bn * 2 <= std::min(forced, cap)) bn *= 2;
        return bn;
    }
    int best = 32; double best_cost = 1e300;
    for (int bn = 32; bn <= cap; bn *= 2) {
        const long items = m_tiles * ((n + bn - 1) / bn);
        const double cost = (double)((items + sms - 1) / sms) * ((double)kblocks * (bn + 64) + 2.0 * bn);
        if (cost < best_cost) { best_cost = cost; best = bn; }
    }
    return best;
}

int grid_cap(int sms, int max_grid) { return max_grid > 0 ? std::min(sms, max_grid) : sms; }

void plan_tiles(TcParams &p, const TcConv &c, bool reg, int sms) {
    const Layer &l = *c.l;
    const bool s2 = l.stride == 2;
    const int esz = elem_size(c.kind), cin = operand_channels(c);
    p.kind = c.kind;
    p.N = c.in.N;
    p.OH = l.out_h; p.OW = l.out_w; p.OHp = c.out.Hp; p.OWp = c.out.Wp;
    p.size = l.size; p.BK = channel_row(cin, esz);
    p.kk = p.BK * esz / 32;
    p.cblocks = cin / p.BK; p.kblocks = l.size * l.size * p.cblocks;
    p.stride2 = s2 ? 1 : 0;
    p.xoff = 1 - l.pad; p.yoff = -l.pad;
    p.PR = s2 ? (c.in.Hp / 2) : c.in.Hp;
    p.row_off = s2 ? 0 : 1;
    const uint32_t row_bytes = 32u * (uint32_t)p.kk;
    p.desc_hi = ((8u * row_bytes) >> 4) | ((row_bytes == 128 ? 1u : row_bytes == 64 ? 2u : 3u) << 30);

    const long rows = (long)p.N * p.PR;
    auto padded = [&](int tw) {
        const int th = 128 / tw;
        return (double)((p.OW + tw - 1) / tw) * tw * (double)((rows + th - 1) / th) * th;
    };
    double best = 1e30; int tw = 1;
    for (int t = 1; t <= 128; t *= 2)
        if (padded(t) < best - 0.5) { best = padded(t); tw = t; }
    if (c.yolo_out) {
        for (int t = 64; t > tw; t /= 2)
            if (padded(t) <= 1.3 * best) { tw = t; break; }
    }
    if (c.pool_mode) tw = 8;
    p.jshift = c.pool_mode ? 1 : 0;
    auto set_tw = [&](int t) {
        p.TW = t; p.TH = 128 / t;
        p.TWlog2 = 0; while ((1 << p.TWlog2) < p.TW) ++p.TWlog2;
        p.xt = (p.OW + p.TW - 1) / p.TW;
        p.jt = (int)((rows - p.jshift + p.TH - 1) / p.TH);
    };
    set_tw(tw);
    p.BN = reg ? pick_bn_reg(l.n, (long)p.xt * p.jt, p.kblocks, sms, c.sw.bn) : pick_bn(l.n);
    if (reg && s2 && p.BN == 32 && p.TW == 1) set_tw(2);
    p.nt = (l.n + p.BN - 1) / p.BN;
    p.num_work = p.xt * p.jt * p.nt;
    p.a_bytes = (uint32_t)(TC_BM * p.BK * esz);
    p.b_bytes = (uint32_t)(p.BN * p.BK * esz);
    p.bstat = (p.nt == 1 && (size_t)p.kblocks * p.b_bytes <= 48 * 1024 && !c.sw.no_bstat) ? 1 : 0;
    p.bstat_bytes = p.bstat ? (uint32_t)p.kblocks * p.b_bytes : 0u;
}

void plan_epilogue(TcParams &p, const TcConv &c, bool reg) {
    const Layer &l = *c.l;
    p.tma_epi = reg ? (p.BN >= 64 ? 64 : 32) : (is_integer(c.kind) && !p.stride2 && !c.acc_out) ? 32 : 0;
    p.stg_bytes = reg ? 2u * 64u * (uint32_t)p.BN * 2u : p.tma_epi ? 2u * 16384u : 4096u * TC_EPI_WARPS;
    p.acc_pitch = p.BN + 4;
    p.out = c.out.base; p.out_ldc = c.out.ldc;
    p.n = l.n;
    p.res = c.res.base;
    p.bias = c.bias; p.act = l.activation; p.act2 = c.act2;
    p.alpha1 = c.alpha1;
    p.mean = c.mean;
    p.xK = l.size * l.size * l.c;
    p.acc_out = c.acc_out;
    p.yolo_out = c.yolo_out;
    p.yolo_per = c.yolo_out ? 4 + c.yolo_classes + 1 : 0;
    p.pool_mode = c.pool_mode; p.pool_mult = c.pool_mult;
    p.pool_out = reinterpret_cast<signed char *>(c.pool_next.base); p.pool_ldc = c.pool_next.ldc;
    p.pool_Hp = c.pool_next.Hp; p.pool_Wp = c.pool_next.Wp;
}

struct TcEpiBytes {
    size_t bias, ymask, stg, acc;
    size_t sum() const { return bias + ymask + stg + acc; }
};
TcEpiBytes epi_bytes(const TcParams &p, bool reg) {
    const size_t f = (size_t)p.nt * p.BN;
    return {sizeof(float) * f,
            reg ? 0 : f / 8,
            p.stg_bytes,
            reg ? 0 : (size_t)TC_BM * p.acc_pitch * sizeof(float)};
}

void plan_ring(TcParams &p, bool reg) {
    const size_t ring_budget = (size_t)(227 - 5) * 1024 - epi_bytes(p, reg).sum();
    const uint32_t ring_blk = p.a_bytes + (p.bstat ? 0u : p.b_bytes);
    p.sps = (int)std::max<uint32_t>(1, std::min<uint32_t>(4, 32u * 1024u / std::max(ring_blk, 1u)));
    p.sps = std::min(p.sps, p.kblocks);
    if (ring_budget < p.bstat_bytes + 2 * (size_t)ring_blk) fatal_throw("tc plan: tile does not fit shared memory");
    const size_t avail = ring_budget - p.bstat_bytes;
    while (p.sps > 1 && avail / ((size_t)p.sps * ring_blk) < 3) --p.sps;
    p.stage_bytes = (uint32_t)p.sps * ring_blk;
    p.stages = (int)std::min<size_t>(8, avail / p.stage_bytes);
    if (p.stages < 2) fatal_throw("tc plan: tile does not fit shared memory");
}

size_t tc_smem_layout(TcParams &p, bool reg) {
    const TcEpiBytes epi = epi_bytes(p, reg);
    size_t top = 0;
    auto place = [&](size_t bytes, size_t align) {
        const size_t off = (top + align - 1) / align * align;
        top = off + bytes;
        return (uint32_t)off;
    };
    if (p.a_bytes % 1024 || p.b_bytes % 1024) fatal_throw("tc plan: operand tiles break the 1024-byte swizzle alignment");
    place(p.bstat_bytes, 1024);
    p.sm.ring = place((size_t)p.stages * p.stage_bytes, 1024);
    const int nbars = 2 * p.stages + 1 + (reg ? 2 * TCR_MAX_SLABS + 2 : 0);
    p.sm.full = place(8 * (size_t)nbars, 8);
    p.sm.empty = p.sm.full + 8u * (uint32_t)p.stages;
    p.sm.bstat_bar = p.sm.empty + 8u * (uint32_t)p.stages;
    p.sm.stg_full = reg ? p.sm.bstat_bar + 8u : 0u;
    p.sm.stg_ready = reg ? p.sm.stg_full + 8u * 2u * TCR_MAX_SLABS : 0u;
    p.sm.bias = place(epi.bias, 16);
    p.sm.ymask = reg ? 0u : place(epi.ymask, 4);
    p.sm.stg = place(epi.stg, p.tma_epi ? 1024 : 128);
    p.sm.acc = reg ? 0u : place(epi.acc, 16);
    const size_t smem = 1024 + top;
    if (smem > 227 * 1024) fatal_throw("tc plan: shared memory budget exceeded");
    return smem;
}

void encode_maps(TcPlan &plan, const TcConv &c, bool reg) {
    const TcParams &p = plan.p;
    const TV &in = c.in;
    const int esz = elem_size(c.kind), cin = operand_channels(c);
    const CUtensorMapSwizzle swz = p.kk == 4 ? CU_TENSOR_MAP_SWIZZLE_128B : p.kk == 2 ? CU_TENSOR_MAP_SWIZZLE_64B : CU_TENSOR_MAP_SWIZZLE_32B;
    const CUtensorMapDataType dtype = c.kind == TC_TF32 ? CU_TENSOR_MAP_DATA_TYPE_FLOAT32
                                    : is_integer(c.kind) ? CU_TENSOR_MAP_DATA_TYPE_UINT8 : CU_TENSOR_MAP_DATA_TYPE_BFLOAT16;
    EncodeTiledFn enc = encode_fn();
    auto check = [](CUresult r, const char *what) {
        if (r != CUDA_SUCCESS) fatal_throw(std::string("cuTensorMapEncodeTiled(") + what + ") failed: " + std::to_string((int)r));
    };
    if (!p.stride2) {
        cuuint64_t dims[3] = {(cuuint64_t)cin, (cuuint64_t)in.Wp, (cuuint64_t)in.N * in.Hp};
        cuuint64_t strides[2] = {(cuuint64_t)in.ldc * esz, (cuuint64_t)in.Wp * in.ldc * esz};
        cuuint32_t box[3] = {(cuuint32_t)p.BK, (cuuint32_t)p.TW, (cuuint32_t)p.TH};
        cuuint32_t es[3] = {1, 1, 1};
        check(enc(&plan.tmA, dtype, 3, in.base, dims, strides, box, es,
                  CU_TENSOR_MAP_INTERLEAVE_NONE, swz, CU_TENSOR_MAP_L2_PROMOTION_L2_128B, CU_TENSOR_MAP_FLOAT_OOB_FILL_NONE), "A");
    } else {
        cuuint64_t dims[5] = {(cuuint64_t)cin, 2, (cuuint64_t)in.Wp / 2, 2, (cuuint64_t)in.N * in.Hp / 2};
        cuuint64_t strides[4] = {(cuuint64_t)in.ldc * esz, (cuuint64_t)in.ldc * 2 * esz, (cuuint64_t)in.Wp * in.ldc * esz,
                                 (cuuint64_t)in.Wp * in.ldc * 2 * esz};
        cuuint32_t box[5] = {(cuuint32_t)p.BK, 1, (cuuint32_t)p.TW, 1, (cuuint32_t)p.TH};
        cuuint32_t es[5] = {1, 1, 1, 1, 1};
        check(enc(&plan.tmA, dtype, 5, in.base, dims, strides, box, es,
                  CU_TENSOR_MAP_INTERLEAVE_NONE, swz, CU_TENSOR_MAP_L2_PROMOTION_L2_128B, CU_TENSOR_MAP_FLOAT_OOB_FILL_NONE), "A");
    }
    {
        const cuuint64_t K = (cuuint64_t)p.size * p.size * cin;
        cuuint64_t dims[2] = {K, (cuuint64_t)c.ldn};
        cuuint64_t strides[1] = {K * esz};
        cuuint32_t box[2] = {(cuuint32_t)p.BK, (cuuint32_t)p.BN};
        cuuint32_t es[2] = {1, 1};
        check(enc(&plan.tmB, dtype, 2, const_cast<void *>(c.w), dims, strides, box, es,
                  CU_TENSOR_MAP_INTERLEAVE_NONE, swz, CU_TENSOR_MAP_L2_PROMOTION_L2_256B, CU_TENSOR_MAP_FLOAT_OOB_FILL_NONE), "B");
    }
    plan.tmO = plan.tmA; plan.tmO1 = plan.tmA; plan.tmR = plan.tmA;
    if (p.tma_epi && c.out.base) {
        const int oesz = c.out_bf16 ? 2 : 4;
        auto encode_px = [&](CUtensorMap *tm, const TV &t, const char *what, int box_rows) {
            cuuint64_t dims[3] = {(cuuint64_t)p.n, (cuuint64_t)t.Wp, (cuuint64_t)t.N * t.Hp};
            cuuint64_t strides[2] = {(cuuint64_t)t.ldc * oesz, (cuuint64_t)t.Wp * t.ldc * oesz};
            cuuint32_t box[3] = {(cuuint32_t)p.tma_epi, (cuuint32_t)std::min(p.TW, reg ? 64 : 128), (cuuint32_t)box_rows};
            cuuint32_t es[3] = {1, 1, 1};
            check(enc(tm, c.out_bf16 ? CU_TENSOR_MAP_DATA_TYPE_BFLOAT16 : CU_TENSOR_MAP_DATA_TYPE_FLOAT32, 3, t.base, dims, strides, box, es,
                      CU_TENSOR_MAP_INTERLEAVE_NONE, p.tma_epi * oesz == 128 ? CU_TENSOR_MAP_SWIZZLE_128B : CU_TENSOR_MAP_SWIZZLE_64B,
                      CU_TENSOR_MAP_L2_PROMOTION_L2_128B, CU_TENSOR_MAP_FLOAT_OOB_FILL_NONE), what);
        };
        const int box_rows = reg ? std::max(p.TH / 2, 1) : p.TH;
        encode_px(&plan.tmO, c.out, "output", box_rows);
        if (reg && p.stride2) encode_px(&plan.tmO1, c.out, "output row", 1);
        if (c.res.base) encode_px(&plan.tmR, c.res, "residual", box_rows);
    }
}

}

int tc_conv_supported(const TcConv &c) {
    const Layer &l = *c.l;
    const bool integer = is_integer(c.kind);
    auto aligned = [](const TV &t, int esz) { return (reinterpret_cast<uintptr_t>(t.base) & 15) == 0 && t.ldc * esz % 16 == 0; };
    if (!geometry_ok(l) || l.n < 8 || (l.activation != YB_LEAKY && l.activation != YB_LINEAR)) return 0;
    if (channel_row(operand_channels(c), elem_size(c.kind)) == 0 || c.in.P != 1 || !aligned(c.in, elem_size(c.kind))) return 0;
    if (c.out_bf16 && (c.kind != TC_BF16 || l.n % 8 != 0)) return 0;
    if (c.out.base ? (c.out.P != 1 || !aligned(c.out, c.out_bf16 ? 2 : 4)) : !(c.yolo_out || c.pool_mode)) return 0;
    if (c.res.base && !(c.kind == TC_BF16 && c.out_bf16 && l.stride == 1 && c.res.H == l.out_h && c.res.W == l.out_w &&
                        c.res.C == l.n && aligned(c.res, 2)))
        return 0;
    if (c.yolo_out && (integer || c.out_bf16)) return 0;
    if (c.pool_mode && !(integer && (c.pool_mode == 1 || c.pool_mode == 2) && !c.acc_out && l.size == 3 && l.stride == 1 &&
                         l.h % 2 == 0 && l.out_h % 2 == 0 && l.out_w % 2 == 0 && l.n % 32 == 0 &&
                         c.pool_next.H == l.out_h / 2 && c.pool_next.W == l.out_w / 2 && aligned(c.pool_next, 1)))
        return 0;
    return 1;
}

TcPlanPtr tc_make_plan(const TcConv &c) {
    const Layer &l = *c.l;
    if (!tc_conv_supported(c)) fatal_throw("tc plan: convolution not supported by the tensor-core kernels");
    TcPlanPtr plan(new TcPlan());
    TcParams &p = plan->p;
    const bool reg = c.kind == TC_BF16 && c.out_bf16;
    const int sms = sm_count();
    plan_tiles(p, c, reg, sms);
    plan_epilogue(p, c, reg);
    plan_ring(p, reg);
    plan->smem = tc_smem_layout(p, reg);
    p.dbg = c.sw.dbg;
    snprintf(plan->desc, sizeof(plan->desc), "%dx%dx%d -> n%d k%d s%d%s", l.c, l.h, l.w, l.n, l.size, l.stride, reg ? " reg" : "");
    encode_maps(*plan, c, reg);
    plan->grid = std::min(p.num_work, grid_cap(sms, c.sw.grid));
    const bool st = c.sw.stats;
    plan->reg = reg;
    if (reg) plan->kernel = st ? k_conv_tc_reg<true> : k_conv_tc_reg<false>;
    else if (is_integer(c.kind)) plan->kernel = st ? k_conv_tc<true, 2> : k_conv_tc<false, 2>;
    else plan->kernel = st ? k_conv_tc<true, 0> : k_conv_tc<false, 0>;
    if (cudaFuncSetAttribute((const void *)plan->kernel, cudaFuncAttributeMaxDynamicSharedMemorySize, 227 * 1024) != cudaSuccess)
        fatal_throw("cudaFuncSetAttribute(k_conv_tc) failed");
    if (st) {
        plan->stats.ensure(TC_NSTATS * (size_t)plan->grid);
        p.stats = plan->stats.get();
        cudaMemset(p.stats, 0, sizeof(unsigned long long) * TC_NSTATS * plan->grid);
    }
    return plan;
}

struct StemPlan { StemTcP p; int grid; bool s2; };
int tc_stem_supported(const Layer &l, const TV &out) {
    return l.c == 3 && l.size == 3 && l.stride == 1 && l.pad == 1 && (l.n == 16 || l.n == 32) &&
           (l.activation == YB_LEAKY || l.activation == YB_LINEAR) && out.base && out.ldc % 8 == 0 &&
           (reinterpret_cast<uintptr_t>(out.base) & 15) == 0;
}
StemPlanPtr tc_stem_make_plan(const Layer &l, const TV &out, const void *d_w, const float *d_bias) {
    StemPlanPtr sp(new StemPlan());
    StemTcP &p = sp->p;
    p.out = out.base; p.out_ldc = out.ldc; p.w = reinterpret_cast<const __nv_bfloat16 *>(d_w); p.bias = d_bias;
    p.N = out.N; p.H = l.h; p.W = l.w; p.OHp = out.Hp; p.OWp = out.Wp; p.nf = l.n; p.act = l.activation;
    p.npix = (long)out.N * l.h * l.w;
    if (p.npix >= (1L << 31) - 256) fatal_throw("stem plan: more than 2^31 pixels per batch");
    p.ntiles = (int)((p.npix + 127) / 128);
    sp->grid = std::min(p.ntiles, sm_count() * 8);
    return sp;
}
int tc_stem_s2_supported(const Layer &l0, const Layer &l1, const TV &out1) {
    return l0.n == 32 && l1.c == 32 && l1.n == 64 && l1.size == 3 && l1.stride == 2 && l1.pad == 1 && l1.h == l0.h && l1.w == l0.w &&
           l0.h % 2 == 0 && l0.w % 2 == 0 && (l1.activation == YB_LEAKY || l1.activation == YB_LINEAR) && out1.base && out1.P == 1 &&
           out1.H == l0.h / 2 && out1.W == l0.w / 2 && out1.ldc % 8 == 0 && (reinterpret_cast<uintptr_t>(out1.base) & 15) == 0;
}
StemPlanPtr tc_stem_s2_make_plan(const Layer &l0, const Layer &l1, const TV &out1, const void *d_w, const float *d_bias,
                                 const void *d_w1, const float *d_bias1, int max_grid) {
    StemPlanPtr sp(new StemPlan());
    sp->s2 = true;
    StemTcP &p = sp->p;
    p.out = out1.base; p.out_ldc = out1.ldc; p.w = reinterpret_cast<const __nv_bfloat16 *>(d_w); p.bias = d_bias;
    p.N = out1.N; p.H = l0.h; p.W = l0.w; p.OHp = out1.Hp; p.OWp = out1.Wp; p.nf = l0.n; p.act = l0.activation;
    p.w1 = reinterpret_cast<const __nv_bfloat16 *>(d_w1); p.bias1 = d_bias1; p.act1 = l1.activation;
    p.OH = out1.H; p.OW = out1.W;
    p.xt = (p.OW + S2_TW - 1) / S2_TW; p.yt = (p.OH + S2_TH - 1) / S2_TH;
    const long ntiles = (long)p.N * p.xt * p.yt;
    if (ntiles >= INT_MAX) fatal_throw("stem plan: too many tiles");
    p.ntiles = (int)ntiles;
    sp->grid = std::min(p.ntiles, grid_cap(2 * sm_count(), max_grid));
    for (const void *f : {(const void *)k_stem_s2_tc<false>, (const void *)k_stem_s2_tc<true>}) {
        if (cudaFuncSetAttribute(f, cudaFuncAttributeMaxDynamicSharedMemorySize, (int)S2_SMEM) != cudaSuccess ||
            cudaFuncSetAttribute(f, cudaFuncAttributePreferredSharedMemoryCarveout, 100) != cudaSuccess)
            fatal_throw("cudaFuncSetAttribute(k_stem_s2_tc) failed");
    }
    return sp;
}
void tc_stem_launch(const StemPlan &sp, const float *d_in_nchw, cudaStream_t s) {
    StemTcP p = sp.p;
    p.in = d_in_nchw;
    if (sp.s2) k_stem_s2_tc<false><<<sp.grid, 256, S2_SMEM, s>>>(p);
    else k_stem_tc<false><<<sp.grid, 128, 0, s>>>(p);
}
void tc_stem_launch_u8(const StemPlan &sp, const unsigned char *d_in_hwc, cudaStream_t s) {
    StemTcP p = sp.p;
    p.in8 = d_in_hwc;
    if (sp.s2) k_stem_s2_tc<true><<<sp.grid, 256, S2_SMEM, s>>>(p);
    else k_stem_tc<true><<<sp.grid, 128, 0, s>>>(p);
}

namespace {
int copy_fields(const int (&f)[TC_PLAN_NFIELDS], int *fields, int n) {
    const int k = std::max(0, std::min(n, (int)TC_PLAN_NFIELDS));
    for (int i = 0; i < k; ++i) fields[i] = f[i];
    return k;
}
}

int tc_plan_fields(const TcPlan &plan, int *fields, int n) {
    const TcParams &p = plan.p;
    const int f[TC_PLAN_NFIELDS] = {plan.reg ? TC_PLAN_CONV_REG : TC_PLAN_CONV, p.kind, p.TW, p.TH, p.BN, p.BK,
                                    p.nt, p.bstat, p.stages, p.sps, plan.grid, p.num_work, p.tma_epi, p.jshift,
                                    p.out ? (int)p.out_ldc : 0};
    return copy_fields(f, fields, n);
}

int tc_stem_plan_fields(const StemPlan &sp, int *fields, int n) {
    const int f[TC_PLAN_NFIELDS] = {sp.s2 ? TC_PLAN_STEM_S2 : TC_PLAN_STEM, TC_BF16, sp.s2 ? S2_TW : -1, sp.s2 ? S2_TH : -1,
                                    sp.s2 ? 64 : -1, -1, -1, -1, -1, -1, sp.grid, sp.p.ntiles, -1, -1, (int)sp.p.out_ldc};
    return copy_fields(f, fields, n);
}

void tc_launch(const TcPlan &P, cudaStream_t s) {
    cudaLaunchConfig_t cfg{};
    cfg.gridDim = dim3((unsigned)P.grid); cfg.blockDim = dim3((unsigned)(P.reg ? TCR_THREADS : TC_THREADS));
    cfg.dynamicSmemBytes = P.smem; cfg.stream = s;
    cudaLaunchAttribute attr[1];
    attr[0].id = cudaLaunchAttributeProgrammaticStreamSerialization;
    attr[0].val.programmaticStreamSerializationAllowed = 1;
    cfg.attrs = attr; cfg.numAttrs = 1;
    cudaLaunchKernelEx(&cfg, P.kernel, P.tmA, P.tmB, P.tmO, P.tmO1, P.tmR, P.p);
}

void TcPlanDelete::operator()(TcPlan *plan) const {
    if (plan->p.stats) {
        std::vector<unsigned long long> h(TC_NSTATS * (size_t)plan->grid);
        cudaDeviceSynchronize();
        cudaMemcpy(h.data(), plan->p.stats, h.size() * sizeof(unsigned long long), cudaMemcpyDeviceToHost);
        double m[TC_NSTATS] = {0};
        for (int b = 0; b < plan->grid; ++b) for (int k = 0; k < TC_NSTATS; ++k) m[k] += (double)h[TC_NSTATS * b + k] / plan->grid;
        fprintf(stderr, "TCSTATS %-28s tiles/cta %.1f kb %d sps %d BN %d | producer: wait_empty %.0f tma_issue %.0f total %.0f | ",
                plan->desc, (double)plan->p.num_work / plan->grid, plan->p.kblocks, plan->p.sps, plan->p.BN,
                m[STAT_PROD_WAIT_EMPTY], m[STAT_PROD_TMA_ISSUE], m[STAT_PROD_TOTAL]);
        if (plan->reg)
            fprintf(stderr, "consumers: wait_full %.0f wait_ready %.0f (first item %.0f) total %.0f | store: wait_full %.0f wait_read %.0f\n",
                    m[STAT_CONS_WAIT_FULL], m[STAT_CONS_WAIT_READY], m[STAT_CONS_FIRST_READY], m[STAT_CONS_TOTAL],
                    m[STAT_STORE_WAIT_FULL], m[STAT_STORE_WAIT_READ]);
        else fprintf(stderr, "consumers: wait_full %.0f total %.0f\n", m[STAT_CONS_WAIT_FULL], m[STAT_CONS_TOTAL]);
    }
    delete plan;
}
void TcPlanDelete::operator()(StemPlan *plan) const { delete plan; }

}
```

### yolo2_light_b200/csrc/yb_conv_tc.cuh

```cuda
#pragma once
#include <cuda_runtime.h>

#include <memory>

#include "yb_kernels.cuh"
#include "yb_model.h"

namespace yb {

enum TcKind {
    TC_BF16 = 0,
    TC_S8 = 1,
    TC_XNOR = 2,
    TC_TF32 = 3,
};

struct TcSwitches {
    int bn = 0;
    int grid = 0;
    bool no_bstat = false;
    bool stats = false;
    int dbg = 0;
};

struct TcConv {
    TcKind kind = TC_BF16;
    const Layer *l = nullptr;
    TV in{};
    TV out{};
    bool out_bf16 = false;
    TV res{};
    int act2 = ACT_LINEAR;
    const void *w = nullptr;
    int ldn = 0;
    const float *bias = nullptr;
    float alpha1 = 0.f;
    const float *mean = nullptr;
    int *acc_out = nullptr;
    float *yolo_out = nullptr;
    int yolo_classes = 0;
    int pool_mode = 0;
    float pool_mult = 0.f;
    TV pool_next{};
    TcSwitches sw{};
};

struct TcPlan;
struct StemPlan;
struct TcPlanDelete {
    void operator()(TcPlan *plan) const;
    void operator()(StemPlan *plan) const;
};
using TcPlanPtr = std::unique_ptr<TcPlan, TcPlanDelete>;
using StemPlanPtr = std::unique_ptr<StemPlan, TcPlanDelete>;

int tc_conv_supported(const TcConv &c);
TcPlanPtr tc_make_plan(const TcConv &c);
void tc_launch(const TcPlan &plan, cudaStream_t s);

int tc_stem_supported(const Layer &l, const TV &out);
StemPlanPtr tc_stem_make_plan(const Layer &l, const TV &out, const void *d_w_32x32_bf16, const float *d_bias);
int tc_stem_s2_supported(const Layer &l0, const Layer &l1, const TV &out1);
StemPlanPtr tc_stem_s2_make_plan(const Layer &l0, const Layer &l1, const TV &out1, const void *d_w_32x32_bf16,
                                 const float *d_bias, const void *d_w1_bf16, const float *d_bias1, int max_grid);
void tc_stem_launch(const StemPlan &plan, const float *d_in_nchw, cudaStream_t s);
void tc_stem_launch_u8(const StemPlan &plan, const unsigned char *d_in_hwc, cudaStream_t s);

enum { TC_PLAN_CONV = 0, TC_PLAN_CONV_REG = 1, TC_PLAN_STEM = 2, TC_PLAN_STEM_S2 = 3, TC_PLAN_NFIELDS = 15 };
int tc_plan_fields(const TcPlan &plan, int *fields, int n);
int tc_stem_plan_fields(const StemPlan &plan, int *fields, int n);

}
```

### yolo2_light_b200/csrc/yb_engine.cu

```cuda
#include "yb_engine.h"

#include <cuda_bf16.h>
#include <cuda_runtime.h>
#include <dlfcn.h>

#include <algorithm>
#include <cmath>
#include <cstdlib>
#include <cstring>

#include "yb_conv_tc.cuh"
#include "yb_cuda.h"
#include "yb_kernels.cuh"
#include "yb_detect.cuh"

namespace yb {

const char *op_kind_name(int k) {
    static const char *names[] = {"input", "conv_simt", "conv_tc", "binarize", "conv_xnor", "quantize",
                                  "conv_int8", "maxpool", "upsample", "shortcut", "route_copy", "reorg",
                                  "yolo", "region", "conv_tc_i8", "conv_tc_tf32"};
    return (k >= 0 && k < 16) ? names[k] : "?";
}

// ... 336 lines not shown
            }
        }
        for (int i = 0; i < nl; ++i)
            if (L[i].has_out && is_alias(i)) L[i].out_dt = L[layer(i).input_layers[0]].out_dt;

        for (int i = 0; i < nl; ++i) {
            if (!is_conv(i)) continue;
            const Layer &l = layer(i);
            LayerPlan &p = L[i];
            if (p.variant == 1 && xnor_fallback(l)) { p.side = SIDE_PM1_F32; p.side_ld = l.c; }
            else if (p.variant == 1 && xnor_on_tc(l)) { p.side = SIDE_S8; p.side_ld = (int)align_up(l.c, 32); }
            else if (p.variant == 1) { p.side = SIDE_BITS; p.side_ld = (l.c + 31) / 32; }
            else if (p.variant == 2) { p.side = SIDE_S8; p.side_ld = (int)align_up(l.c, 32); }
        }

        for (int i = 0; i < nl; ++i)
            if (is_conv(i)) L[i].path = conv_path(i);
        plan_first_op();
        plan_fusions();
        for (int i = 0; i < nl; ++i)
            if (is_alias(i)) L[i].materialised = L[i].has_out && L[layer(i).input_layers[0]].materialised;
        reject_unsupported();
    }

    void reject_unsupported() const {
        for (int i = 0; i < nl; ++i) {
            const Layer &l = layer(i);
            const LayerPlan &p = L[i];
            const bool reads_prev = l.type == YB_CONVOLUTIONAL || l.type == YB_MAXPOOL || l.type == YB_UPSAMPLE || l.type == YB_REORG ||
                                    l.type == YB_YOLO || l.type == YB_REGION || (l.type == YB_SHORTCUT && !p.fused_sc);
            if (reads_prev && i > 0 && !L[i - 1].has_out) fatal_throw("engine: layer " + std::to_string(i) + " has no image input");
            switch (l.type) {
            case YB_CONVOLUTIONAL: {
                if (!L[p.fused_into >= 0 ? p.fused_into : i].has_out) fatal_throw("engine: conv output not placed");
                const int in_c = i == 0 ? net.c : layer(i - 1).out_c, in_h = i == 0 ? net.h : layer(i - 1).out_h,
                          in_w = i == 0 ? net.w : layer(i - 1).out_w;
                if (in_c != l.c || in_h != l.h || in_w != l.w) fatal_throw("engine: conv input shape mismatch");
                break;
            }
            case YB_UPSAMPLE:
                if (l.reverse) fatal_throw("engine: reverse upsample (downsample) is not supported");
                break;
            case YB_REORG:
                if (l.reverse) fatal_throw("engine: reverse reorg is not supported");
                break;
            case YB_SHORTCUT:
                if (!L[l.index].materialised) fatal_throw("engine: shortcut source not placed");
                break;
            case YB_ROUTE:
                if (!p.has_out) fatal_throw("engine: route over layers of different spatial size is not supported");
                if (is_alias(i)) break;
                for (int j : l.input_layers)
                    if (L[j].owner != i && !L[j].materialised) fatal_throw("engine: route source not placed");
                break;
            default:
                break;
            }
        }
    }

    int conv_path(int i) const {
        const Layer &l = layer(i);
        const LayerPlan &p = L[i];
        const int tgt = p.fused_into >= 0 ? p.fused_into : i;
        const TV tin = layout_in(i), tout = layout_view(tgt);
        const int idt = in_dt(i), odt = L[tgt].out_dt;
        const TcConv tc_query = tc_conv(i, false, 0);
        if (p.variant == 0) {
            int tc = (ADT == DT_BF16 && idt == DT_BF16) ? tc_conv_supported(tc_query) : 0;
            if (ADT == DT_F32 && opt.precision == YB_PREC_BF16_TC && idt == DT_F32 && odt == DT_F32 && p.fused_into < 0 &&
                !cons[i].empty() && !sw.no_tf32) {
                bool heads_only = true;
                for (int r : cons[i]) heads_only &= layer(r).type == YB_YOLO || layer(r).type == YB_REGION;
                if (heads_only && tc_conv_supported(tc_query)) tc = 2;
            }
            if (sw.no_tc) tc = 0;
            return tc == 2 ? CP_TF32 : tc ? CP_TC : CP_SIMT;
        }
        if (idt != DT_F32 || odt != DT_F32)
            fatal_throw(p.variant == 1 ? "engine: xnor path needs f32 activations" : "engine: int8 path needs f32 activations");
        if (p.variant == 2) return (!sw.no_tc && tc_conv_supported(tc_query)) ? CP_I8_TC : CP_I8_SIMT;
        if (xnor_fallback(l)) return CP_XNOR_FALLBACK;
        if (xnor_on_tc(l) && vec4_view(tin)) {
            if (!tc_conv_supported(tc_query)) fatal_throw("engine: xnor tensor-core layer not supported by the i8 tile");
            return CP_XNOR_TC;
        }
        const int CW = p.side_ld;
        if (CW <= 2 && l.size == 3 && (size_t)l.n * 9 * CW * 4 <= 40 * 1024 && tout.ldc % 4 == 0) return CP_XNOR_SMALLK;
        return CP_XNOR_GENERAL;
    }

    void plan_first_op() {
        const Layer &l0 = layer(0);
        const TV out0 = layout_view(0);
        const bool stem_ok = l0.type == YB_CONVOLUTIONAL && L[0].variant == 0 && L[0].path == CP_SIMT && l0.c == 3 &&
                             l0.size == 3 && l0.stride == 1 && l0.pad == 1 && (l0.n == 16 || l0.n == 32) && L[0].fused_into < 0 &&
                             L[0].has_out && !sw.no_stem && (L[0].out_dt == DT_F32 || out0.ldc % 8 == 0);
        bool pool_ok = stem_ok && opt.fuse && L[0].out_dt == DT_F32 && l0.n == 16 && nl > 2 && !sw.no_stem_pool_fuse &&
                       (l0.activation == YB_LEAKY || l0.activation == YB_LINEAR);
        if (pool_ok) {
            const Layer &mp = layer(1), &c2 = layer(2);
            pool_ok = mp.type == YB_MAXPOOL && mp.size == 2 && mp.stride == 2 && mp.pad == 1 && sole_reader(0, 1) &&
                      sole_reader(1, 2) && c2.type == YB_CONVOLUTIONAL && L[2].variant != 0 && L[2].side != SIDE_NONE &&
                      !xnor_fallback(c2) && (L[2].side == SIDE_BITS || L[2].side_ld % 16 == 0);
        }
        if (pool_ok) {
            first = FIRST_STEM_POOL;
        } else if (stem_ok && L[0].out_dt == DT_BF16 && tc_stem_supported(l0, out0) && !sw.no_stem_tc) {
            const bool s2 = opt.fuse && !sw.no_stem_s2_fuse && nl > 1 && sole_reader(0, 1) && is_conv(1) && L[1].variant == 0 &&
                            L[1].path == CP_TC && L[1].fused_into < 0 && L[1].out_dt == DT_BF16 &&
                            tc_stem_s2_supported(l0, layer(1), layout_view(1));
            first = s2 ? FIRST_STEM_S2 : FIRST_STEM_TC;
        } else if (stem_ok) {
            first = FIRST_STEM_SIMT;
        }
        if (first != FIRST_NHWC) L[0].in_first_op = true;
        if (first == FIRST_STEM_S2 || first == FIRST_STEM_POOL) {
            L[0].materialised = false;
            L[1].in_first_op = true;
        }
        if (first == FIRST_STEM_POOL) {
            L[1].materialised = false;
            L[2].prefilled = true;
        }
    }

    void plan_fusions() {
        for (int i = 0; i < nl; ++i) {
            LayerPlan &p = L[i];
            if (!is_conv(i) || p.in_first_op) continue;
            const int pm = conv_pool_mode(i);
            bool pool = false;
            if (p.path == CP_XNOR_TC || p.path == CP_I8_TC) {
                pool = pm != 0 && tc_conv_supported(tc_conv(i, false, pm));
            } else if (p.path == CP_XNOR_SMALLK) {
                pool = pm == 2 || pm == 3;
            }
            if (pool) {
                p.pool_mode = pm;
                L[i + 1].pool_in_conv = L[i + 2].prefilled = true;
                p.materialised = L[i + 1].materialised = false;
            }
            if ((p.path == CP_TF32 || p.path == CP_TC) && opt.fuse && p.fused_into < 0 && p.out_dt == DT_F32 && i + 1 < nl &&
                layer(i + 1).type == YB_YOLO && sole_reader(i, i + 1) && !sw.no_yolo_fuse) {
                p.yolo_fused = L[i + 1].yolo_fused = true;
                p.materialised = false;
            }
        }
        for (int i = 0; i + 1 < nl; ++i) {
            if (layer(i).type != YB_MAXPOOL || L[i].in_first_op || L[i].pool_in_conv) continue;
            const Layer &c = layer(i + 1);
            if (opt.fuse && in_dt(i) == DT_F32 && sole_reader(i, i + 1) && c.type == YB_CONVOLUTIONAL && L[i + 1].variant != 0 &&
                L[i + 1].side != SIDE_NONE && !xnor_fallback(c) && !sw.no_pool_fuse) {
                L[i].pool_to_side = L[i + 1].prefilled = true;
                L[i].materialised = false;
            }
        }
    }

    void place() {
        size_t total = 0;
        auto take = [&](size_t bytes) { const size_t off = total; total += align_up(bytes, 1024); return off; };
        const size_t in0_off = first == FIRST_NHWC ? take(tv_bytes(B, net.h, net.w, net.c, P, ADT)) : 0;
        for (int i = 0; i < nl; ++i) {
            const Layer &l = layer(i);
            if (L[i].materialised && !is_alias(i) && L[i].owner < 0)
                buf_off[i] = take(tv_bytes(B, l.out_h, l.out_w, L[i].ldc, P, L[i].out_dt));
        }
        for (int i = 0; i < nl; ++i) {
            const Layer &l = layer(i);
            const int sdt = L[i].side == SIDE_PM1_F32 ? DT_F32 : L[i].side == SIDE_S8 ? DT_S8 : DT_BITS;
            if (L[i].side != SIDE_NONE) side_off[i] = take(tv_bytes(B, l.h, l.w, L[i].side_ld, P, sdt));
        }
        e.act_arena.ensure(total);
        CUDA_OK(cudaMemsetAsync(e.act_arena.get(), 0, total, e.stream));
        for (int i = 0; i < nl; ++i)
            if (L[i].variant == 1 && L[i].side == SIDE_S8)
                CUDA_OK(cudaMemsetAsync(e.act_arena.get() + side_off[i], 0xFF, tv_bytes(B, layer(i).h, layer(i).w, L[i].side_ld, P, DT_S8), e.stream));
        e.in0 = first == FIRST_NHWC ? in0_view(e.act_arena.get() + in0_off) : TV{};
        e.in0_dt = ADT;
        e.act_dt = ADT;
        e.out_tv.assign(nl, TV{});
        e.out_dt.assign(nl, ADT);
        for (int i = 0; i < nl; ++i) {
            e.out_dt[i] = L[i].out_dt;
            if (L[i].materialised) e.out_tv[i] = out_view(i, [&](int j) { return e.act_arena.get() + buf_off[j]; });
        }
    }

    void place_finals() {
        e.finals.resize(nl);
        e.counts.resize(nl);
        for (int i = 0; i < nl; ++i) {
            const Layer &l = layer(i);
            if (!(l.type == YB_YOLO || l.type == YB_REGION || (i == nl - 1 && l.outputs > 0))) continue;
            e.finals[i].d.ensure((size_t)l.outputs * B);
            e.finals[i].h.ensure((size_t)l.outputs * B);
        }
    }

    void pack_weights() {
        std::vector<char> hostw;
        auto reserve = [&](size_t bytes) { size_t off = align_up(hostw.size(), 1024); hostw.resize(off + bytes, 0); return off; };
        for (int i = 0; i < nl; ++i) {
            if (!is_conv(i)) continue;
            const Layer &l = layer(i);
            const LayerPlan &p = L[i];
            const int taps = l.size * l.size, K = taps * l.c;
            ConvWeights &w = cw[i];
            w.bias = reserve(sizeof(float) * align_up(l.n, 64));
            memcpy(&hostw[w.bias], l.biases.data(), sizeof(float) * l.n);
            w.ldn = (int)align_up(l.n, 64);
            if (p.path == CP_TF32) {
                w.w_f32km = reserve(sizeof(float) * (size_t)w.ldn * K);
                float *dst = reinterpret_cast<float *>(&hostw[w.w_f32km]);
                for_each_weight(l, [&](int f, int c, int t, size_t k) { dst[(size_t)f * K + (size_t)t * l.c + c] = l.weights[k]; });
            } else if (p.path == CP_TC) {
                w.w_bf16 = reserve(sizeof(__nv_bfloat16) * (size_t)w.ldn * K);
                __nv_bfloat16 *dst = reinterpret_cast<__nv_bfloat16 *>(&hostw[w.w_bf16]);
                for_each_weight(l, [&](int f, int c, int t, size_t k) {
                    dst[(size_t)f * K + (size_t)t * l.c + c] = __float2bfloat16_rn(l.weights[k]); });
            } else if (p.variant == 0) {
                w.ldw = w.ldn;
                w.w_f32 = reserve(sizeof(float) * (size_t)K * w.ldw);
                float *dst = reinterpret_cast<float *>(&hostw[w.w_f32]);
                for_each_weight(l, [&](int f, int c, int t, size_t k) {
                    dst[(ADT == DT_F32 ? (size_t)c * taps + t : (size_t)t * l.c + c) * w.ldw + f] = l.weights[k]; });
            } else if (p.side == SIDE_PM1_F32) {
                w.ldw = w.ldn;
                w.w_f32 = reserve(sizeof(float) * (size_t)K * w.ldw);
                float *dst = reinterpret_cast<float *>(&hostw[w.w_f32]);
                for_each_weight(l, [&](int f, int c, int t, size_t k) {
                    dst[((size_t)c * taps + t) * w.ldw + f] = l.weights[k] > 0 ? l.mean_arr[f] : -l.mean_arr[f]; });
            } else if (p.side == SIDE_BITS) {
                const int CW = p.side_ld;
                w.cpad = CW * 32;
                w.w_bits = reserve(sizeof(uint32_t) * (size_t)w.ldn * taps * CW);
                uint32_t *dst = reinterpret_cast<uint32_t *>(&hostw[w.w_bits]);
                for_each_weight(l, [&](int f, int c, int t, size_t k) {
                    if (l.weights[k] > 0) dst[((size_t)f * taps + t) * CW + c / 32] |= 1u << (c & 31); });
            } else {
                w.cpad = p.side_ld;
                w.w_s8 = reserve((size_t)w.ldn * taps * w.cpad);
                int8_t *dst = reinterpret_cast<int8_t *>(&hostw[w.w_s8]);
                for_each_weight(l, [&](int f, int c, int t, size_t k) {
                    dst[((size_t)f * taps + t) * w.cpad + c] = p.variant == 2 ? l.weights_int8[k] : l.weights[k] > 0 ? 1 : -1; });
            }
            if (p.variant == 1 && p.side != SIDE_PM1_F32) {
                w.mean = reserve(sizeof(float) * align_up(l.n, 64));
                memcpy(&hostw[w.mean], l.mean_arr.data(), sizeof(float) * l.n);
            }
        }
        if (first == FIRST_STEM_TC || first == FIRST_STEM_S2) {
            stem_w_off = reserve(sizeof(__nv_bfloat16) * 32 * 32);
            __nv_bfloat16 *dst = reinterpret_cast<__nv_bfloat16 *>(&hostw[stem_w_off]);
            for (int k = 0; k < 32 * 32; ++k) dst[k] = __float2bfloat16_rn(0.f);
            const Layer &l0 = layer(0);
            for_each_weight(l0, [&](int f, int c, int t, size_t k) { dst[f * 32 + t * 3 + c] = __float2bfloat16_rn(l0.weights[k]); });
        }
        e.w_arena.ensure(align_up(std::max<size_t>(hostw.size(), 1024), 1024));
        if (opt.upload) CUDA_OK(cudaMemcpyAsync(e.w_arena.get(), hostw.data(), hostw.size(), cudaMemcpyHostToDevice, e.stream));
        CUDA_OK(cudaStreamSynchronize(e.stream));
    }

    const float *bias(int i) const { return reinterpret_cast<const float *>(e.w_arena.get() + cw[i].bias); }
    void push(int kind, int i, std::function<void(const float *, cudaStream_t)> f) { e.ops.push_back(Op{kind, i, std::move(f), nullptr}); }
    template <typename... A>
    void push_kernel(int kind, int i, void (*k)(A...), dim3 grid, dim3 block, size_t smem, typename same_type<A>::type... args) {
        push(kind, i, [=](const float *, cudaStream_t s) { k<<<grid, block, smem, s>>>(args...); });
    }
    template <typename... A>
    void push_input_kernel(int kind, int i, void (*k)(const float *, A...), dim3 grid, dim3 block, typename same_type<A>::type... args) {
        push(kind, i, [=](const float *in, cudaStream_t s) { k<<<grid, block, 0, s>>>(in, args...); });
    }

    void push_tc_plan(int kind, int i) {
        e.tc_plans.emplace_back(i, tc_make_plan(tc_conv(i, true, L[i].pool_mode)));
        const TcPlan *plan = e.tc_plans.back().second.get();
        if (kind == OP_CONV_TC || kind == OP_CONV_TC_TF32) ++e.n_tc;
        push(kind, i, [plan](const float *, cudaStream_t s) { tc_launch(*plan, s); });
    }

    int32_t *counts_buffer(int i) {
        if (!opt.keep_counts) return nullptr;
        const Layer &l = layer(i);
        e.counts[i].ensure((size_t)B * l.n * l.out_h * l.out_w);
        return e.counts[i].get();
    }

    void emit_first() {
        const Layer &l0 = layer(0);
        const int act = l0.activation, H = l0.h, W = l0.w;
        if (first == FIRST_STEM_POOL) {
            decltype(&k_stem_pool<0, ACT_LEAKY>) const k[3][2] = {{k_stem_pool<0, ACT_LEAKY>, k_stem_pool<0, ACT_LINEAR>},
                                                                  {k_stem_pool<1, ACT_LEAKY>, k_stem_pool<1, ACT_LINEAR>},
                                                                  {k_stem_pool<2, ACT_LEAKY>, k_stem_pool<2, ACT_LINEAR>}};
            const Layer &c2 = layer(2);
            const int mode = L[2].variant == 2 ? 0 : L[2].side == SIDE_S8 ? 1 : 2;
            push_input_kernel(OP_CONV_SIMT, 0, k[mode][act == ACT_LEAKY ? 0 : 1], (unsigned)(((long)B * c2.h * c2.w + 127) / 128), 128,
                              side_placed(2), stem_weights<16>(l0), act, H, W, mode == 0 ? c2.input_quant_multipler : 0.f);
        } else if (first == FIRST_STEM_TC || first == FIRST_STEM_S2) {
            const bool s2 = first == FIRST_STEM_S2;
            e.stem_plan = s2 ? tc_stem_s2_make_plan(l0, layer(1), e.out_tv[1], e.w_arena.get() + stem_w_off, bias(0),
                                                    e.w_arena.get() + cw[1].w_bf16, bias(1), sw.tc.grid)
                             : tc_stem_make_plan(l0, e.out_tv[0], e.w_arena.get() + stem_w_off, bias(0));
            const StemPlan *sp = e.stem_plan.get();
            if (s2) ++e.n_tc;
            push(OP_CONV_TC, s2 ? 1 : 0, [sp](const float *in, cudaStream_t s) { tc_stem_launch(*sp, in, s); });
            if (!sw.no_stem_u8) e.ops[0].launch_u8 = [sp](const unsigned char *in, cudaStream_t s) { tc_stem_launch_u8(*sp, in, s); };
        } else if (first == FIRST_STEM_SIMT) {
            const bool bf16 = L[0].out_dt == DT_BF16;
            const unsigned grid = (unsigned)(((long)B * H * W + 127) / 128);
            if (l0.n == 32)
                push_input_kernel(OP_CONV_SIMT, 0, bf16 ? k_conv_stem<32, __nv_bfloat16> : k_conv_stem<32, float, true>, grid, 128,
                                  e.out_tv[0], stem_weights<32>(l0), act, H, W);
            else
                push_input_kernel(OP_CONV_SIMT, 0, bf16 ? k_conv_stem<16, __nv_bfloat16> : k_conv_stem<16, float, true>, grid, 128,
                                  e.out_tv[0], stem_weights<16>(l0), act, H, W);
        } else {
            push_input_kernel(OP_INPUT, -1, BY_DT(k_input_nchw_to_nhwc, ADT), grid_for((long)e.in0.N * e.in0.H * e.in0.W), 256, e.in0);
        }
    }

    void emit_conv(int i) {
        const TV tin = i == 0 ? e.in0 : e.out_tv[i - 1];
        if (L[i].variant == 0) emit_conv_fp32(i, tin);
        else if (L[i].variant == 1) emit_conv_xnor(i, tin);
        else emit_conv_int8(i, tin);
    }

    void push_conv_simt(int i, void (*k)(ConvP), const TV &tin, const TV &tout, const TV &res, int act2) {
        const Layer &l = layer(i);
        const long M = (long)B * l.out_h * l.out_w;
        ConvP cp{};
        cp.in = tin; cp.out = tout; cp.res = res;
        cp.w = e.w_arena.get() + cw[i].w_f32;
        cp.bias = bias(i);
        cp.n = l.n; cp.ldw = cw[i].ldw; cp.size = l.size; cp.stride = l.stride; cp.pad = l.pad;
        cp.act = l.activation; cp.act2 = act2; cp.K = l.size * l.size * l.c; cp.M = M;
        push_kernel(OP_CONV_SIMT, i, k, dim3((unsigned)((M + 63) / 64), (unsigned)((l.n + 63) / 64)), 256, 0, cp);
    }

    void emit_conv_fp32(int i, const TV &tin) {
        const LayerPlan &p = L[i];
        if (p.path == CP_TC || p.path == CP_TF32) {
            push_tc_plan(p.path == CP_TC ? OP_CONV_TC : OP_CONV_TC_TF32, i);
            return;
        }
        const int tgt = p.fused_into >= 0 ? p.fused_into : i;
        TV res{}; int rdt = DT_F32; int act2 = ACT_LINEAR;
        if (p.fused_into >= 0) {
            const Layer &s = layer(tgt);
            res = e.out_tv[s.index];
            rdt = L[s.index].out_dt;
            act2 = s.activation;
        }
        void (*const k[2][2][2])(ConvP) = {
            {{k_conv_simt<float, float, float, true>, k_conv_simt<float, float, __nv_bfloat16>},
             {k_conv_simt<float, __nv_bfloat16, float>, k_conv_simt<float, __nv_bfloat16, __nv_bfloat16>}},
            {{k_conv_simt<__nv_bfloat16, float, float>, k_conv_simt<__nv_bfloat16, float, __nv_bfloat16>},
             {k_conv_simt<__nv_bfloat16, __nv_bfloat16, float>, k_conv_simt<__nv_bfloat16, __nv_bfloat16, __nv_bfloat16>}}};
        push_conv_simt(i, k[in_dt(i)][L[tgt].out_dt][rdt], tin, e.out_tv[tgt], res, act2);
    }

    void emit_conv_xnor(int i, const TV &tin) {
        const Layer &l = layer(i);
        const LayerPlan &p = L[i];
        const TV tout = e.out_tv[i];
        const long M = (long)B * l.out_h * l.out_w;
        if (p.path == CP_XNOR_FALLBACK) {
            const TV pm1 = side_placed(i);
            push_kernel(OP_BINARIZE, i, k_binarize_pm1, grid_for((long)B * l.h * l.w * l.c), 256, 0, tin, pm1);
            push_conv_simt(i, k_conv_simt<float, float, float, true>, pm1, tout, TV{}, ACT_LINEAR);
            return;
        }
        int32_t *cnt_dbg = counts_buffer(i);
        if (p.path == CP_XNOR_TC) {
            if (!p.prefilled)
                push_kernel(OP_BINARIZE, i, k_binarize_s8, grid_for((long)B * l.h * l.w * (l.c / 16)), 256, 0, tin, side_placed(i));
            push_tc_plan(OP_CONV_TC_I8, i);
            return;
        }
        const int CW = p.side_ld;
        const TV bits = make_tv(e.act_arena.get() + side_off[i], B, l.h, l.w, CW, CW, P, DT_BITS, 0);
        if (!p.prefilled) {
            const bool vec = vec4_view(tin);
            push_kernel(OP_BINARIZE, i, vec ? k_binarize_vec<float> : k_binarize<float>,
                        grid_for((long)B * l.h * l.w * CW * (vec ? 1 : 32)), 256, 0, tin, bits);
        }
        XnorP xp{};
        xp.bits = bits; xp.out = tout;
        xp.w = reinterpret_cast<const uint32_t *>(e.w_arena.get() + cw[i].w_bits);
        xp.mean = reinterpret_cast<const float *>(e.w_arena.get() + cw[i].mean);
        xp.bias = bias(i);
        xp.n = l.n; xp.size = l.size; xp.pad = l.pad; xp.K = l.size * l.size * l.c;
        xp.padbits = (CW * 32 - l.c) * l.size * l.size;
        xp.act = l.activation; xp.M = M; xp.counts = cnt_dbg;
        if (p.path == CP_XNOR_GENERAL) {
            push_kernel(OP_CONV_XNOR, i, k_conv_xnor, dim3((unsigned)((M + 63) / 64), (unsigned)((l.n + 63) / 64)), 256, 0, xp);
            return;
        }
        const size_t smem = (size_t)l.n * 9 * CW * 4;
        if (const int pm = p.pool_mode) {
            void (*const k[2][2])(XnorP, TV) = {{k_conv_xnor_smallk_pool<1, 2>, k_conv_xnor_smallk_pool<1, 3>},
                                                {k_conv_xnor_smallk_pool<2, 2>, k_conv_xnor_smallk_pool<2, 3>}};
            xp.out = make_tv(nullptr, B, l.out_h, l.out_w, l.n, L[i].ldc, P, DT_F32, 0);
            const Layer &c2 = layer(i + 2);
            push_kernel(OP_CONV_XNOR, i, k[CW - 1][pm - 2], (unsigned)(((long)B * c2.h * c2.w + 127) / 128), 128, smem, xp,
                        side_placed(i + 2));
            return;
        }
        push_kernel(OP_CONV_XNOR, i, CW == 1 ? k_conv_xnor_smallk<1> : k_conv_xnor_smallk<2>, (unsigned)((M + 127) / 128), 128, smem, xp);
    }

    void emit_conv_int8(int i, const TV &tin) {
        const Layer &l = layer(i);
        const LayerPlan &p = L[i];
        const TV tout = e.out_tv[i];
        const TV q = side_placed(i);
        if (!p.prefilled)
            push_kernel(OP_QUANTIZE, i, k_quantize<float>, grid_for((long)B * l.h * l.w * (p.side_ld / 4)), 256, 0, tin, q,
                        l.input_quant_multipler);
        int *acc_dbg = counts_buffer(i);
        if (p.path == CP_I8_TC) {
            push_tc_plan(OP_CONV_TC_I8, i);
            return;
        }
        const long M = (long)B * l.out_h * l.out_w;
        Int8P ip{};
        ip.q = q; ip.out = tout;
        ip.w = reinterpret_cast<const uint32_t *>(e.w_arena.get() + cw[i].w_s8);
        ip.bias = bias(i);
        ip.alpha1 = alpha1(l);
        ip.n = l.n; ip.size = l.size; ip.stride = l.stride; ip.pad = l.pad; ip.act = l.activation;
        ip.CW = p.side_ld / 4; ip.M = M; ip.acc_out = acc_dbg;
        push_kernel(OP_CONV_INT8, i, k_conv_int8_simt, dim3((unsigned)((M + 63) / 64), (unsigned)((l.n + 63) / 64)), 256, 0, ip);
    }

    void emit_small(int i) {
        const Layer &l = layer(i);
        const LayerPlan &p = L[i];
        const TV tin = i == 0 ? e.in0 : e.out_tv[i - 1];
        const int dt = in_dt(i);
        const TV tout = e.out_tv[i];
        const int g = grid_for((long)B * l.out_h * l.out_w * l.out_c);
        switch (l.type) {
        case YB_MAXPOOL: {
            if (p.pool_in_conv) break;
            if (p.pool_to_side) {
                void (*const k[3])(TV, TV, int, int, int, float) = {k_maxpool_fused<0>, k_maxpool_fused<1>, k_maxpool_fused<2>};
                const Layer &c = layer(i + 1);
                const TV q = side_placed(i + 1);
                const int mode = L[i + 1].side == SIDE_BITS ? 2 : L[i + 1].variant == 2 ? 0 : 1;
                push_kernel(OP_MAXPOOL, i, k[mode], grid_for((long)B * c.h * c.w * (mode == 2 ? q.ldc : q.ldc / 4)), 256, 0, tin, q,
                            l.size, l.stride, l.pad, mode == 0 ? c.input_quant_multipler : 0.f);
                break;
            }
            const int esz = (int)dt_size(dt);
            const bool vec = (l.out_c * esz) % 16 == 0 && (tin.ldc * esz) % 16 == 0 && (tout.ldc * esz) % 16 == 0 &&
                             (reinterpret_cast<uintptr_t>(tin.base) & 15) == 0 && (reinterpret_cast<uintptr_t>(tout.base) & 15) == 0;
            const int gv = grid_for((long)B * l.out_h * l.out_w * ((l.out_c * esz) / 16 + 1));
            push_kernel(OP_MAXPOOL, i, vec ? BY_DT(k_maxpool_vec, dt) : BY_DT(k_maxpool, dt), vec ? gv : g, 256, 0, tin, tout, l.size,
                        l.stride, l.pad);
            break;
        }
        case YB_UPSAMPLE: {
            const int esz = (int)dt_size(dt);
            const bool vec = l.scale == 1.f && (l.out_c * esz) % 16 == 0 && (tin.ldc * esz) % 16 == 0 && (tout.ldc * esz) % 16 == 0 &&
                             (reinterpret_cast<uintptr_t>(tin.base) & 15) == 0 && (reinterpret_cast<uintptr_t>(tout.base) & 15) == 0;
            if (vec)
                push_kernel(OP_UPSAMPLE, i, k_upsample_vec16, grid_for((long)B * l.out_h * l.out_w * ((l.out_c * esz) / 16 + 1)), 256, 0,
                            tin, tout, l.stride, esz);
            else
                push_kernel(OP_UPSAMPLE, i, BY_DT(k_upsample, dt), g, 256, 0, tin, tout, l.stride, l.scale);
            break;
        }
        case YB_SHORTCUT: {
            if (p.fused_sc) break;
            const int stride = std::max(l.w / l.out_w, 1), sample = std::max(l.out_w / l.w, 1);
            const int minw = std::min(l.w, l.out_w), minh = std::min(l.h, l.out_h), minc = std::min(l.c, l.out_c);
            push_kernel(OP_SHORTCUT, i, BY_DT(k_shortcut, dt), g, 256, 0, tin, e.out_tv[l.index], tout, stride, sample, minw, minh,
                        minc, l.activation);
            break;
        }
        case YB_ROUTE: {
            if (is_alias(i)) break;
            int off = 0;
            for (int j : l.input_layers) {
                const Layer &src = layer(j);
                if (L[j].owner != i) {
                    TV slice = tout;
                    slice.base += (size_t)off * dt_size(p.out_dt);
                    slice.C = src.out_c;
                    push_kernel(OP_ROUTE_COPY, i, BY_DT(k_copy_channels, p.out_dt),
                                grid_for((long)B * src.out_h * src.out_w * src.out_c), 256, 0, e.out_tv[j], slice);
                }
                off += src.out_c;
            }
            break;
        }
        case YB_REORG:
            push_kernel(OP_REORG, i, BY_DT(k_reorg, dt), g, 256, 0, tin, tout, l.stride);
            break;
        case YB_YOLO:
            if (p.yolo_fused) break;
            push_kernel(OP_YOLO, i, BY_DT(k_yolo, dt), grid_for((long)B * ((l.h * l.w + 31) / 32) * ((l.c + 31) / 32) * 256), 256, 0,
                        tin, e.finals[i].d.get(), l.classes, ADT == DT_BF16 ? 1 : 0);
            break;
        case YB_REGION:
            push_kernel(OP_REGION, i, BY_DT(k_region, dt), grid_for((long)B * l.h * l.w * l.n), 256, 0, tin, e.finals[i].d.get(), l.n,
                        l.classes, l.coords, l.softmax);
            break;
        default:
            break;
        }
    }

    void emit_last_copy() {
        const int last = nl - 1;
        const Layer &l = layer(last);
        if (l.type == YB_YOLO || l.type == YB_REGION || !e.finals[last].d) return;
        const int src = L[last].fused_into >= 0 ? L[last].fused_into : last;
        const TV t = e.out_tv[src];
        if (!t.base) return;
        push_kernel(OP_YOLO, last, BY_DT(k_nhwc_to_nchw_f32, L[src].out_dt), grid_for((long)B * l.outputs), 256, 0, t,
                    e.finals[last].d.get());
    }

    void emit_ops() {
        emit_first();
        for (int i = 0; i < nl; ++i) {
            if (L[i].in_first_op) continue;
            if (is_conv(i)) emit_conv(i);
            else emit_small(i);
        }
        emit_last_copy();
    }
};
}

std::shared_ptr<Engine> build_engine(Network *net, const EngineOptions &opt) {
    int ndev = 0;
    if (cudaGetDeviceCount(&ndev) != cudaSuccess || ndev == 0)
        fatal_throw("yolo2_light_b200: no CUDA device -- this library has no CPU fallback");
    CUDA_OK(cudaSetDevice(opt.device));
    cudaDeviceProp prop;
    CUDA_OK(cudaGetDeviceProperties(&prop, opt.device));
    if (prop.major != 9 || prop.minor != 0)
        fatal_throw(std::string("yolo2_light_b200: device '") + prop.name + "' is compute capability " +
                    std::to_string(prop.major) + "." + std::to_string(prop.minor) +
                    "; this build contains sm_90a code only");
    if (net->layers.empty()) fatal_throw("empty network");

    auto e = std::make_shared<Engine>();
    e->opt = opt;
    e->batch = net->batch;
    e->sw = Switches::read();
    e->opt.fuse = opt.fuse && !e->sw.no_fuse;
    e->stream = make_stream();

    Builder b(*net, *e);
    b.plan_layers();
    b.place();
    b.place_finals();
    b.pack_weights();
    e->d_input.ensure((size_t)net->batch * net->c * net->h * net->w);
    b.emit_ops();
    CUDA_OK(cudaStreamSynchronize(e->stream));
    CUDA_OK(cudaGetLastError());
    return e;
}

static void engine_forward_impl(Engine *e, const void *d_input, const unsigned char *d_u8_frames, void *stream);
void engine_forward(Engine *e, const void *d_input, void *stream) { engine_forward_impl(e, d_input, nullptr, stream); }

void engine_upload_input(Engine *e, const float *host_input, void *stream) {
    cudaStream_t s = stream ? (cudaStream_t)stream : (cudaStream_t)e->stream;
    CUDA_OK(cudaSetDevice(e->opt.device));
    CUDA_OK(cudaMemcpyAsync(e->d_input.get(), host_input, e->d_input.count() * sizeof(float), cudaMemcpyHostToDevice, s));
}

static void fill_geo(Engine *e, Engine::FrameStage &st, const Network *net, const int *w, const int *h, int nimg, int letter) {
    const int B = e->batch;
    st.h_geo.ensure(B);
    st.d_geo.ensure(B);
    for (int b = 0; b < B; ++b) {
        ImageGeo &g = st.h_geo.get()[b];
        g = ImageGeo{};
        if (b >= nimg) continue;
        g.w = w[b]; g.h = h[b];
        int lw, lh;
        letterbox_size(net->w, net->h, g.w, g.h, &lw, &lh);
        g.new_w = letter ? lw : net->w; g.new_h = letter ? lh : net->h;
        g.nw = net->letterbox ? lw : net->w; g.nh = net->letterbox ? lh : net->h;
        g.dx = (net->w - g.nw) / 2; g.dy = (net->h - g.nh) / 2;
        g.w_scale = (float)(g.w - 1) / (float)(g.nw - 1);
        g.h_scale = (float)(g.h - 1) / (float)(g.nh - 1);
    }
}

static void launch_resize(Engine *e, const Engine::FrameStage &st, const Network *net, int nimg, int fmt, float *dst,
                          cudaStream_t s) {
    if (!e->d_unit) {
        float unit[256];
        for (int v = 0; v < 256; ++v) unit[v] = (float)((double)(float)v / 255.);
        DevBuf<float> d_unit(256);
        CUDA_OK(cudaMemcpy(d_unit.get(), unit, sizeof(unit), cudaMemcpyHostToDevice));
// ... 467 lines not shown
```

Before: 3202.

## Warp-specialize fused stem+layer1 kernel with double-buffered im2col and TMA stores

Restructures the fused stride-2 stem plus layer-1 kernel into 384 threads. Two warpgroups build the stem im2col rows and run the stem MMA, and a third warpgroup consumes them for layer 1. Handoff goes through double-buffered shared sets guarded by full/empty mbarriers, and output is written with 4D TMA stores from double-buffered staging tiles. It also precomputes per-thread patch and scatter offsets, adds an interior fast path that skips bounds checks, and adds optional cycle stats. The cost is one block per SM instead of two, more shared memory, and more complex synchronisation.

```diff
diff --git a/yolo2_light_b200/csrc/yb_conv_tc.cu b/yolo2_light_b200/csrc/yb_conv_tc.cu
--- a/yolo2_light_b200/csrc/yb_conv_tc.cu
+++ b/yolo2_light_b200/csrc/yb_conv_tc.cu
@@ -138,8 +138,13 @@
     asm volatile("cp.async.bulk.tensor.3d.global.shared::cta.bulk_group [%0, {%2, %3, %4}], [%1];"
                  ::"l"(tm), "r"(src), "r"(c0), "r"(c1), "r"(c2) : "memory");
 }
+__device__ __forceinline__ void tma_store_4d(const CUtensorMap *tm, uint32_t src, int c0, int c1, int c2, int c3) {
+    asm volatile("cp.async.bulk.tensor.4d.global.shared::cta.bulk_group [%0, {%2, %3, %4, %5}], [%1];"
+                 ::"l"(tm), "r"(src), "r"(c0), "r"(c1), "r"(c2), "r"(c3) : "memory");
+}
 __device__ __forceinline__ void tma_store_commit() { asm volatile("cp.async.bulk.commit_group;" ::: "memory"); }
 __device__ __forceinline__ void tma_store_wait_read0() { asm volatile("cp.async.bulk.wait_group.read 0;" ::: "memory"); }
+__device__ __forceinline__ void tma_store_wait_read1() { asm volatile("cp.async.bulk.wait_group.read 1;" ::: "memory"); }
 __device__ __forceinline__ void tma_store_wait_all() { asm volatile("cp.async.bulk.wait_group 0;" ::: "memory"); }
 __device__ __forceinline__ void named_bar_sync(int id, int nthreads) {
     asm volatile("bar.sync %0, %1;" ::"r"(id), "r"(nthreads) : "memory");
@@ -353,7 +358,8 @@
     STAT_STORE_WAIT_READ,
     TC_NSTATS = 16
 };
-__device__ __forceinline__ unsigned long long &tc_stat(const TcParams &p, TcStat s) { return p.stats[blockIdx.x * TC_NSTATS + s]; }
+template <typename P>
+__device__ __forceinline__ unsigned long long &tc_stat(const P &p, TcStat s) { return p.stats[blockIdx.x * TC_NSTATS + s]; }
 template <bool ST, typename F>
 __device__ __forceinline__ void timed(long long &cycles, F &&f) {
     if constexpr (ST) { const long long c0 = clock64(); f(); cycles += clock64() - c0; }
@@ -919,6 +925,7 @@
     const __nv_bfloat16 *w1;
     const float *bias1;
     int act1, OH, OW, xt, yt;
+    unsigned long long *stats;
 };
 
 template <bool U8>
@@ -1070,203 +1077,292 @@
 
 constexpr int S2_TW = 16, S2_TH = 8;
 constexpr int S2_RW = 2 * S2_TW + 1, S2_RH = 2 * S2_TH + 1;
+constexpr int S2_PIX = S2_RW * S2_RH;
 constexpr int S2_ROWS = 640;
+constexpr int S2_PH = S2_RH + 2, S2_PW = S2_RW + 2, S2_PP = 36;
+constexpr int S2_PATCH = 3 * S2_PH * S2_PW;
+constexpr int S2_THREADS = 384;
+constexpr uint32_t S2_SETS_KX = 17u * 1024u;
+constexpr uint32_t S2_DUMP = 3u * S2_SETS_KX;
+constexpr uint32_t S2_U_BYTES = S2_DUMP + 1024u;
+constexpr uint32_t S2_STG_BYTES = 128u * 128u;
 constexpr uint32_t S2_B1 = 0;
 constexpr uint32_t S2_BS = 9u * 4096u;
 constexpr uint32_t S2_U = S2_BS + 2048u;
-constexpr uint32_t S2_SETS_KX = 17u * 1024u;
-constexpr uint32_t S2_STG = (uint32_t)S2_ROWS * 64u;
-constexpr uint32_t S2_MISC = S2_U + S2_STG + 2u * 8192u;
-constexpr int S2_PH = S2_RH + 2, S2_PW = S2_RW + 2, S2_PP = 36;
+constexpr uint32_t S2_STG = S2_U + 2u * S2_U_BYTES;
+constexpr uint32_t S2_BAR = S2_STG + 2u * S2_STG_BYTES;
+constexpr uint32_t S2_MISC = S2_BAR + 4u * 8u;
 constexpr size_t S2_SMEM = 1024 + S2_MISC + 4 * (32 + 64 + 256) + 4 * 3 * S2_PH * S2_PP;
-static_assert(S2_STG + 2u * 8192u >= 3u * S2_SETS_KX, "sets must fit the shared region");
-
-template <bool U8>
-__global__ void __launch_bounds__(256, 2) k_stem_s2_tc(StemTcP p) {
+static_assert(S2_U_BYTES >= (uint32_t)S2_ROWS * 64u, "the im2col rows must fit a sets buffer");
+static_assert(S2_U % 1024 == 0 && S2_U_BYTES % 1024 == 0 && S2_STG % 1024 == 0, "wgmma operands and staging tiles: 1 KB aligned");
+static_assert(S2_SMEM <= 227 * 1024, "shared memory per block");
+
+template <bool U8, bool ST>
+__global__ void __launch_bounds__(S2_THREADS, 1) k_stem_s2_tc(const __grid_constant__ CUtensorMap tmO, const StemTcP p) {
     extern __shared__ uint8_t smem_raw[];
-    uint8_t *sm = smem_raw + ((1024u - (smem_u32(smem_raw) & 1023u)) & 1023u);
-    const uint32_t base = smem_u32(sm), U = base + S2_U;
+    const uint32_t base = smem_base(smem_raw);
+    uint8_t *sm = static_cast<uint8_t *>(smem_ptr(base));
     float *bias0_s = reinterpret_cast<float *>(sm + S2_MISC), *bias1_s = bias0_s + 32, *lut = bias1_s + 64, *patch = lut + 256;
+    const uint32_t full = base + S2_BAR, empty = full + 16u;
     const int t = threadIdx.x, lane = t & 31;
     const int warp = __shfl_sync(0xffffffffu, t >> 5, 0), wg = warp >> 2;
-    if constexpr (U8) lut[t] = (float)((double)(float)t / 255.0);
+    if constexpr (U8) { if (t < 256) lut[t] = (float)((double)(float)t / 255.0); }
     if (t < 32) bias0_s[t] = p.bias[t];
     if (t < 64) bias1_s[t] = p.bias1[t];
     if (t < 128) {
         const int f = t >> 2, j = t & 3;
         *reinterpret_cast<uint4 *>(sm + S2_BS + f * 64 + ((j ^ ((f >> 1) & 3)) << 4)) = *reinterpret_cast<const uint4 *>(p.w + f * 32 + j * 8);
     }
-    for (int i = t; i < 9 * 64 * 4; i += 256) {
+    for (int i = t; i < 9 * 64 * 4; i += S2_THREADS) {
         const int r = i >> 8, f = (i >> 2) & 63, j = i & 3;
         *reinterpret_cast<uint4 *>(sm + S2_B1 + r * 4096 + f * 64 + ((j ^ ((f >> 1) & 3)) << 4)) =
             *reinterpret_cast<const uint4 *>(p.w1 + f * 288 + r * 32 + j * 8);
     }
+    if (t == 0) {
+        for (int b = 0; b < 2; ++b) { mbar_init(full + 8u * b, 8); mbar_init(empty + 8u * b, 4); }
+        fence_mbar_init();
+    }
+    if (t == 256) prefetch_tmap(&tmO);
     asm volatile("fence.proxy.async.shared::cta;" ::: "memory");
     __syncthreads();
 
     const uint32_t hi = ((8u * 64u) >> 4) | (2u << 30);
-    const bool leaky0 = p.act == ACT_LEAKY, leaky1 = p.act1 == ACT_LEAKY;
     const int rl = 16 * (warp & 3) + (lane >> 2), cq = 2 * (lane & 3);
-    constexpr int PER = (3 * S2_PH * S2_PW + 255) / 256;
-    auto patch_index = [&](int e, int &c, int &r, int &col) {
-        if constexpr (U8) { r = e / (3 * S2_PW); const int b = e - r * 3 * S2_PW; col = b / 3; c = b - col * 3; }
-        else { c = e / (S2_PH * S2_PW); const int b = e - c * S2_PH * S2_PW; r = b / S2_PW; col = b - r * S2_PW; }
+    auto tile_pos = [&](int tile, int &n, int &ox0, int &oy0) {
+        const int tx = tile % p.xt, rest = tile / p.xt, ty = rest % p.yt;
+        n = rest / p.yt; ox0 = tx * S2_TW; oy0 = ty * S2_TH;
     };
-    auto load_patch = [&](int tile, float (&v)[PER]) {
-        const int tx = tile % p.xt, rest = tile / p.xt, ty = rest % p.yt, n = rest / p.yt;
-        const int py0 = 2 * ty * S2_TH - 2, px0 = 2 * tx * S2_TW - 2;
-        const size_t img = (size_t)n * 3 * p.H * p.W;
+    const long long t_begin = ST ? clock64() : 0;
+
+    if (wg < 2) {
+        constexpr int PER = (S2_PATCH + 255) / 256;
+        uint32_t pk[PER];
+        int goff[PER];
 #pragma unroll
         for (int k = 0; k < PER; ++k) {
             const int e = t + 256 * k;
             int c, r, col;
-            patch_index(e, c, r, col);
-            const int y = py0 + r, x = px0 + col;
-            const bool in_img = e < 3 * S2_PH * S2_PW && y >= 0 && y < p.H && x >= 0 && x < p.W;
-            if constexpr (U8) v[k] = in_img ? lut[__ldg(p.in8 + img + (unsigned)((y * p.W + x) * 3 + c))] : 0.f;
-            else v[k] = in_img ? __ldg(p.in + img + (unsigned)((c * p.H + y) * p.W + x)) : 0.f;
-        }
-    };
-    float pv[PER];
-    if ((int)blockIdx.x < p.ntiles) load_patch(blockIdx.x, pv);
-    for (int tile = blockIdx.x; tile < p.ntiles; tile += gridDim.x) {
-        const int tx = tile % p.xt, rest = tile / p.xt, ty = rest % p.yt, n = rest / p.yt;
-        const int ox0 = tx * S2_TW, oy0 = ty * S2_TH;
-        const int gy0 = 2 * oy0 - 1, gx0 = 2 * ox0 - 1;
-
-#pragma unroll
-        for (int k = 0; k < PER; ++k) {
-            const int e = t + 256 * k;
-            if (e >= 3 * S2_PH * S2_PW) break;
-            int c, r, col;
-            patch_index(e, c, r, col);
-            patch[(c * S2_PH + r) * S2_PP + col] = pv[k];
-        }
-        __syncthreads();
-
-        for (int i = t; i < S2_ROWS; i += 256) {
-            const int sy = i / S2_RW, sx = i - sy * S2_RW;
-            const float *w0 = patch + sy * S2_PP + sx;
-            const bool ok = i < S2_RW * S2_RH;
-            uint32_t packed[16];
-            {
-                float v[32];
-#pragma unroll
-                for (int ky = 0; ky < 3; ++ky)
-#pragma unroll
-                    for (int kx = 0; kx < 3; ++kx)
-#pragma unroll
-                        for (int c = 0; c < 3; ++c) v[(ky * 3 + kx) * 3 + c] = ok ? w0[(c * S2_PH + ky) * S2_PP + kx] : 0.f;
-#pragma unroll
-                for (int k = 27; k < 32; ++k) v[k] = 0.f;
-#pragma unroll
-                for (int k = 0; k < 16; ++k) packed[k] = pack_bf16x2(v[2 * k], v[2 * k + 1]);
+            if constexpr (U8) { r = e / (3 * S2_PW); const int b = e - r * 3 * S2_PW; col = b / 3; c = b - col * 3; }
+            else { c = e / (S2_PH * S2_PW); const int b = e - c * S2_PH * S2_PW; r = b / S2_PW; col = b - r * S2_PW; }
+            pk[k] = e < S2_PATCH ? (uint32_t)((c * S2_PH + r) * S2_PP + col) | (uint32_t)r << 12 | (uint32_t)col << 17 : 0x80000000u;
+            goff[k] = U8 ? (r * p.W + col) * 3 + c : (c * p.H + r) * p.W + col;
+        }
+        int woff[3];
+#pragma unroll
+        for (int k = 0; k < 3; ++k) {
+            const int i = t + 256 * k, sy = i / S2_RW, sx = i - sy * S2_RW;
+            woff[k] = i < S2_PIX ? sy * S2_PP + sx : -1;
+        }
+        uint32_t putA[10], putB[10];
+#pragma unroll
+        for (int c = 0; c < 5; ++c)
+#pragma unroll
+            for (int h = 0; h < 2; ++h) {
+                const int i = 64 * (5 * wg + c) + rl + 8 * h, sy = i / S2_RW, sx = i - sy * S2_RW;
+                const uint32_t set = ((sy & 1) ? 9u * 1024u : 0u) + (uint32_t)(sy >> 1) * 1024u + 2u * (uint32_t)cq;
+                auto row = [&](int kx, int ox) { return set + (uint32_t)kx * S2_SETS_KX + (uint32_t)ox * 64u + ((uint32_t)((ox >> 1) & 3) << 4); };
+                const bool odd = sx & 1, last = sx == 2 * S2_TW;
+                putA[2 * c + h] = i < S2_PIX ? row(odd ? 1 : last ? 2 : 0, last ? (sx >> 1) - 1 : sx >> 1) | (uint32_t)sy << 17 | (uint32_t)sx << 22 : S2_DUMP;
+                putB[2 * c + h] = i < S2_PIX && !odd && !last && sx >= 2 ? row(2, (sx >> 1) - 1) : S2_DUMP;
             }
-#pragma unroll
-            for (int j = 0; j < 4; ++j)
-                *reinterpret_cast<uint4 *>(sm + S2_U + i * 64 + ((j ^ ((i >> 1) & 3)) << 4)) =
-                    make_uint4(packed[4 * j], packed[4 * j + 1], packed[4 * j + 2], packed[4 * j + 3]);
-        }
-        asm volatile("fence.proxy.async.shared::cta;" ::: "memory");
-        __syncthreads();
-
-        float ds[5][16];
-#pragma unroll
-        for (int c = 0; c < 5; ++c)
-#pragma unroll
-            for (int i = 0; i < 16; ++i) ds[c][i] = 0.f;
-#pragma unroll
-        for (int c = 0; c < 5; ++c) wg_fence_operand(ds[c]);
-        wg_fence();
-#pragma unroll
-        for (int c = 0; c < 5; ++c)
-#pragma unroll
-            for (int k = 0; k < 2; ++k)
-                Wg<TC_BF16, 32>::mma(ds[c], wg_desc(U + (uint32_t)(5 * wg + c) * 4096u + 32u * k, hi), wg_desc(base + S2_BS + 32u * k, hi), (uint32_t)k);
-        wg_commit();
-        wg_wait<0>();
-#pragma unroll
-        for (int c = 0; c < 5; ++c) wg_fence_operand(ds[c]);
-        __syncthreads();
-
-        {
+
+        using PV = typename std::conditional<U8, uint32_t, float>::type;
+        PV pv[PER];
+        auto load_patch = [&](int tile) {
+            int n, ox0, oy0;
+            tile_pos(tile, n, ox0, oy0);
+            const int py0 = 2 * oy0 - 2, px0 = 2 * ox0 - 2;
+            const size_t img = (size_t)n * 3 * p.H * p.W;
+            const int off0 = U8 ? (py0 * p.W + px0) * 3 : py0 * p.W + px0;
+            auto ld = [&](int k) -> PV {
+                if constexpr (U8) return __ldg(p.in8 + img + (unsigned)(off0 + goff[k]));
+                else return __ldg(p.in + img + (unsigned)(off0 + goff[k]));
+            };
+            if (py0 >= 0 && px0 >= 0 && py0 + S2_PH <= p.H && px0 + S2_PW <= p.W) {
+#pragma unroll
+                for (int k = 0; k < PER; ++k) pv[k] = (k < PER - 1 || !(pk[k] >> 31)) ? ld(k) : PV(0);
+            } else {
+#pragma unroll
+                for (int k = 0; k < PER; ++k) {
+                    const int y = py0 + (int)((pk[k] >> 12) & 31u), x = px0 + (int)((pk[k] >> 17) & 63u);
+                    pv[k] = !(pk[k] >> 31) && (unsigned)y < (unsigned)p.H && (unsigned)x < (unsigned)p.W ? ld(k) : PV(0);
+                }
+            }
+        };
+        const bool leaky0 = p.act == ACT_LEAKY;
+        long long w_empty = 0;
+        if ((int)blockIdx.x < p.ntiles) load_patch(blockIdx.x);
+        int j = 0;
+        for (int tile = blockIdx.x; tile < p.ntiles; tile += gridDim.x, ++j) {
+            const uint32_t b = (uint32_t)j & 1u, U = base + S2_U + b * S2_U_BYTES;
+            uint8_t *u = sm + S2_U + b * S2_U_BYTES;
+            int n, ox0, oy0;
+            tile_pos(tile, n, ox0, oy0);
+            const int gy0 = 2 * oy0 - 1, gx0 = 2 * ox0 - 1;
+
+#pragma unroll
+            for (int k = 0; k < PER; ++k) {
+                if (pk[k] >> 31) continue;
+                if constexpr (U8) patch[pk[k] & 0xFFFu] = lut[pv[k]];
+                else patch[pk[k] & 0xFFFu] = pv[k];
+            }
+            named_bar_sync(1, 256);
+            if (tile + (int)gridDim.x < p.ntiles) load_patch(tile + gridDim.x);
+
+            timed<ST>(w_empty, [&] { mbar_wait(empty + 8u * b, ((uint32_t)j >> 1 & 1u) ^ 1u); });
+#pragma unroll
+            for (int k = 0; k < 3; ++k) {
+                if (woff[k] < 0) continue;
+                const int i = t + 256 * k;
+                const float *w0 = patch + woff[k];
+                uint32_t packed[16];
+                {
+                    float v[32];
+#pragma unroll
+                    for (int ky = 0; ky < 3; ++ky)
+#pragma unroll
+                        for (int kx = 0; kx < 3; ++kx)
+#pragma unroll
+                            for (int c = 0; c < 3; ++c) v[(ky * 3 + kx) * 3 + c] = w0[(c * S2_PH + ky) * S2_PP + kx];
+#pragma unroll
+                    for (int q = 27; q < 32; ++q) v[q] = 0.f;
+#pragma unroll
+                    for (int q = 0; q < 16; ++q) packed[q] = pack_bf16x2(v[2 * q], v[2 * q + 1]);
+                }
+#pragma unroll
+                for (int q = 0; q < 4; ++q)
+                    *reinterpret_cast<uint4 *>(u + i * 64 + ((q ^ ((i >> 1) & 3)) << 4)) =
+                        make_uint4(packed[4 * q], packed[4 * q + 1], packed[4 * q + 2], packed[4 * q + 3]);
+            }
+            asm volatile("fence.proxy.async.shared::cta;" ::: "memory");
+            named_bar_sync(1, 256);
+
+            float ds[5][16];
 #pragma unroll
             for (int c = 0; c < 5; ++c)
 #pragma unroll
-                for (int h = 0; h < 2; ++h) {
-                    const int i = 64 * (5 * wg + c) + rl + 8 * h;
-                    if (i >= S2_RW * S2_RH) continue;
-                    const int sy = i / S2_RW, sx = i - sy * S2_RW, y = gy0 + sy, x = gx0 + sx;
-                    const bool in_img = y >= 0 && y < p.H && x >= 0 && x < p.W;
-                    uint32_t v[4];
-#pragma unroll
-                    for (int j = 0; j < 4; ++j) {
-                        float a = ds[c][4 * j + 2 * h] + bias0_s[8 * j + cq], b = ds[c][4 * j + 2 * h + 1] + bias0_s[8 * j + cq + 1];
-                        if (leaky0) { a = fmaxf(a, 0.1f * a); b = fmaxf(b, 0.1f * b); }
-                        v[j] = in_img ? pack_bf16x2(a, b) : 0u;
+                for (int i = 0; i < 16; ++i) ds[c][i] = 0.f;
+#pragma unroll
+            for (int c = 0; c < 5; ++c) wg_fence_operand(ds[c]);
+            wg_fence();
+#pragma unroll
+            for (int c = 0; c < 5; ++c)
+#pragma unroll
+                for (int k = 0; k < 2; ++k)
+                    Wg<TC_BF16, 32>::mma(ds[c], wg_desc(U + (uint32_t)(5 * wg + c) * 4096u + 32u * k, hi), wg_desc(base + S2_BS + 32u * k, hi), (uint32_t)k);
+            wg_commit();
+            wg_wait<0>();
+#pragma unroll
+            for (int c = 0; c < 5; ++c) wg_fence_operand(ds[c]);
+            named_bar_sync(1, 256);
+
+            float b0[8];
+#pragma unroll
+            for (int q = 0; q < 4; ++q) { b0[2 * q] = bias0_s[8 * q + cq]; b0[2 * q + 1] = bias0_s[8 * q + cq + 1]; }
+            auto epilogue = [&](auto inside_c) {
+#pragma unroll
+                for (int c = 0; c < 5; ++c)
+#pragma unroll
+                    for (int h = 0; h < 2; ++h) {
+                        const uint32_t pa = putA[2 * c + h], pb = putB[2 * c + h];
+                        bool in_img = true;
+                        if constexpr (!decltype(inside_c)::value) {
+                            const int y = gy0 + (int)((pa >> 17) & 31u), x = gx0 + (int)((pa >> 22) & 63u);
+                            in_img = (unsigned)y < (unsigned)p.H && (unsigned)x < (unsigned)p.W;
+                        }
+                        uint32_t v[4];
+#pragma unroll
+                        for (int q = 0; q < 4; ++q) {
+                            float a = ds[c][4 * q + 2 * h] + b0[2 * q], e = ds[c][4 * q + 2 * h + 1] + b0[2 * q + 1];
+                            if (leaky0) { a = fmaxf(a, 0.1f * a); e = fmaxf(e, 0.1f * e); }
+                            v[q] = in_img ? pack_bf16x2(a, e) : 0u;
+                        }
+                        auto put = [&](uint32_t row) {
+#pragma unroll
+                            for (int q = 0; q < 4; ++q) asm volatile("st.shared.b32 [%0], %1;" ::"r"(row ^ ((uint32_t)q << 4)), "r"(v[q]));
+                        };
+                        put(U + (pa & 0x1FFFFu));
+                        put(U + pb);
                     }
-                    const uint32_t set = U + ((sy & 1) ? 9u * 1024u : 0u) + (uint32_t)(sy >> 1) * 1024u + 2u * (uint32_t)cq;
-                    auto put = [&](int kx, int ox) {
-                        const uint32_t row = set + (uint32_t)kx * S2_SETS_KX + (uint32_t)ox * 64u;
-#pragma unroll
-                        for (int j = 0; j < 4; ++j)
-                            asm volatile("st.shared.b32 [%0], %1;" ::"r"(row + ((uint32_t)(j ^ ((ox >> 1) & 3)) << 4)), "r"(v[j]));
-                    };
-                    const bool odd = sx & 1, last = sx == 2 * S2_TW;
-                    put(odd ? 1 : last ? 2 : 0, last ? (sx >> 1) - 1 : sx >> 1);
-                    if (!odd && !last && sx >= 2) put(2, (sx >> 1) - 1);
-                }
-        }
-        asm volatile("fence.proxy.async.shared::cta;" ::: "memory");
-        __syncthreads();
-
-        if (tile + (int)gridDim.x < p.ntiles) load_patch(tile + gridDim.x, pv);
-
-        float d[32];
-#pragma unroll
-        for (int i = 0; i < 32; ++i) d[i] = 0.f;
-        wg_fence_operand(d);
-        wg_fence();
-#pragma unroll
-        for (int r = 0; r < 9; ++r) {
-            const int ky = r / 3, kx = r % 3;
-            const uint32_t a = U + (uint32_t)kx * S2_SETS_KX + ((ky & 1) ? 9u * 1024u : 0u) + (uint32_t)(ky >> 1) * 1024u + (uint32_t)wg * 4096u;
-            const uint32_t b = base + S2_B1 + (uint32_t)r * 4096u;
-#pragma unroll
-            for (int k = 0; k < 2; ++k)
-                Wg<TC_BF16, 64>::mma(d, wg_desc(a + 32u * k, hi), wg_desc(b + 32u * k, hi), (r > 0 || k > 0) ? 1u : 0u);
-        }
-        wg_commit();
-        wg_wait<0>();
-        wg_fence_operand(d);
-        __syncthreads();
-
-        const uint32_t stg = U + S2_STG + (uint32_t)wg * 8192u;
+            };
+            if (gy0 >= 0 && gx0 >= 0 && gy0 + S2_RH <= p.H && gx0 + S2_RW <= p.W) epilogue(std::true_type{});
+            else epilogue(std::false_type{});
+            asm volatile("fence.proxy.async.shared::cta;" ::: "memory");
+            __syncwarp();
+            if (lane == 0) mbar_arrive(full + 8u * b);
+        }
+        if (ST && p.stats && t == 0) {
+            tc_stat(p, STAT_PROD_WAIT_EMPTY) = w_empty;
+            tc_stat(p, STAT_PROD_TOTAL) = clock64() - t_begin;
+        }
+    } else {
+        const int lt = t - 256;
+        const bool leaky1 = p.act1 == ACT_LEAKY;
         float b1[16];
 #pragma unroll
-        for (int j = 0; j < 8; ++j) { b1[2 * j] = bias1_s[8 * j + cq]; b1[2 * j + 1] = bias1_s[8 * j + cq + 1]; }
-#pragma unroll
-        for (int h = 0; h < 2; ++h) {
-            const int q = rl + 8 * h;
-#pragma unroll
-            for (int j = 0; j < 8; ++j) {
-                float a = d[4 * j + 2 * h] + b1[2 * j], b = d[4 * j + 2 * h + 1] + b1[2 * j + 1];
-                if (leaky1) { a = fmaxf(a, 0.1f * a); b = fmaxf(b, 0.1f * b); }
-                asm volatile("st.shared.b32 [%0], %1;" ::"r"(stg + (uint32_t)q * 128u + ((uint32_t)(j ^ (q & 7)) << 4) + 2u * (uint32_t)cq),
-                             "r"(pack_bf16x2(a, b)) : "memory");
+        for (int q = 0; q < 8; ++q) { b1[2 * q] = bias1_s[8 * q + cq]; b1[2 * q + 1] = bias1_s[8 * q + cq + 1]; }
+        long long w_full = 0, w_read = 0;
+        int j = 0;
+        for (int tile = blockIdx.x; tile < p.ntiles; tile += gridDim.x, ++j) {
+            const uint32_t b = (uint32_t)j & 1u, U = base + S2_U + b * S2_U_BYTES;
+            int n, ox0, oy0;
+            tile_pos(tile, n, ox0, oy0);
+            timed<ST>(w_full, [&] { mbar_wait(full + 8u * b, (uint32_t)j >> 1 & 1u); });
+
+            float d[2][32];
+#pragma unroll
+            for (int h = 0; h < 2; ++h) {
+#pragma unroll
+                for (int i = 0; i < 32; ++i) d[h][i] = 0.f;
+                wg_fence_operand(d[h]);
             }
-        }
-        if (wg == 0) named_bar_sync(1, 128);
-        else named_bar_sync(2, 128);
-#pragma unroll
-        for (int k = 0; k < 4; ++k) {
-            const int idx = (t & 127) + 128 * k, q = idx >> 3, ch = idx & 7;
-            const int oy = oy0 + 4 * wg + (q >> 4), ox = ox0 + (q & 15);
-            if (oy < p.OH && ox < p.OW) {
-                uint4 o;
-                asm volatile("ld.shared.v4.b32 {%0, %1, %2, %3}, [%4];" : "=r"(o.x), "=r"(o.y), "=r"(o.z), "=r"(o.w)
-                             : "r"(stg + (uint32_t)q * 128u + ((uint32_t)(ch ^ (q & 7)) << 4)) : "memory");
-                *reinterpret_cast<uint4 *>(p.out + ((size_t)(n * p.OHp + oy + 1) * p.OWp + ox + 1) * (size_t)p.out_ldc * 2 + ch * 16) = o;
+            wg_fence();
+#pragma unroll
+            for (int r = 0; r < 9; ++r) {
+                const int ky = r / 3, kx = r % 3;
+                const uint32_t a = U + (uint32_t)kx * S2_SETS_KX + ((ky & 1) ? 9u * 1024u : 0u) + (uint32_t)(ky >> 1) * 1024u;
+                const uint32_t bw = base + S2_B1 + (uint32_t)r * 4096u;
+#pragma unroll
+                for (int k = 0; k < 2; ++k)
+#pragma unroll
+                    for (int h = 0; h < 2; ++h)
+                        Wg<TC_BF16, 64>::mma(d[h], wg_desc(a + (uint32_t)h * 4096u + 32u * k, hi), wg_desc(bw + 32u * k, hi), (r > 0 || k > 0) ? 1u : 0u);
+            }
+            wg_commit();
+            wg_wait<0>();
+#pragma unroll
+            for (int h = 0; h < 2; ++h) wg_fence_operand(d[h]);
+            __syncwarp();
+            if (lane == 0) mbar_arrive(empty + 8u * b);
+
+            const uint32_t stg = base + S2_STG + b * S2_STG_BYTES;
+            if (lt == 0) timed<ST>(w_read, tma_store_wait_read1);
+            named_bar_sync(2, 128);
+#pragma unroll
+            for (int h = 0; h < 2; ++h)
+#pragma unroll
+                for (int hh = 0; hh < 2; ++hh) {
+                    const int r = 64 * h + rl + 8 * hh;
+#pragma unroll
+                    for (int q = 0; q < 8; ++q) {
+                        float a = d[h][4 * q + 2 * hh] + b1[2 * q], e = d[h][4 * q + 2 * hh + 1] + b1[2 * q + 1];
+                        if (leaky1) { a = fmaxf(a, 0.1f * a); e = fmaxf(e, 0.1f * e); }
+                        asm volatile("st.shared.b32 [%0], %1;" ::"r"(stg + (uint32_t)r * 128u + ((uint32_t)(q ^ (r & 7)) << 4) + 2u * (uint32_t)cq),
+                                     "r"(pack_bf16x2(a, e)) : "memory");
+                    }
+                }
+            asm volatile("fence.proxy.async.shared::cta;" ::: "memory");
+            named_bar_sync(2, 128);
+            if (lt == 0) {
+                tma_store_4d(&tmO, stg, 0, ox0, oy0, n);
+                tma_store_commit();
+            }
+        }
+        if (lt == 0) {
+            tma_store_wait_all();
+            if (ST && p.stats) {
+                tc_stat(p, STAT_CONS_WAIT_FULL) = w_full; tc_stat(p, STAT_STORE_WAIT_READ) = w_read;
+                tc_stat(p, STAT_CONS_TOTAL) = clock64() - t_begin;
             }
         }
     }
@@ -1286,6 +1382,14 @@
         fn = reinterpret_cast<EncodeTiledFn>(p);
     }
     return fn;
+}
+
+void encode_tiled(CUtensorMap *tm, CUtensorMapDataType dtype, int rank, void *base, const cuuint64_t *dims, const cuuint64_t *strides,
+                  const cuuint32_t *box, CUtensorMapSwizzle swz, CUtensorMapL2promotion promo, const char *what) {
+    const cuuint32_t es[5] = {1, 1, 1, 1, 1};
+    const CUresult r = encode_fn()(tm, dtype, (cuuint32_t)rank, base, dims, strides, box, es, CU_TENSOR_MAP_INTERLEAVE_NONE, swz, promo,
+                                   CU_TENSOR_MAP_FLOAT_OOB_FILL_NONE);
+    if (r != CUDA_SUCCESS) fatal_throw(std::string("cuTensorMapEncodeTiled(") + what + ") failed: " + std::to_string((int)r));
 }
 
 }
@@ -1473,34 +1577,24 @@
     const CUtensorMapSwizzle swz = p.kk == 4 ? CU_TENSOR_MAP_SWIZZLE_128B : p.kk == 2 ? CU_TENSOR_MAP_SWIZZLE_64B : CU_TENSOR_MAP_SWIZZLE_32B;
     const CUtensorMapDataType dtype = c.kind == TC_TF32 ? CU_TENSOR_MAP_DATA_TYPE_FLOAT32
                                     : is_integer(c.kind) ? CU_TENSOR_MAP_DATA_TYPE_UINT8 : CU_TENSOR_MAP_DATA_TYPE_BFLOAT16;
-    EncodeTiledFn enc = encode_fn();
-    auto check = [](CUresult r, const char *what) {
-        if (r != CUDA_SUCCESS) fatal_throw(std::string("cuTensorMapEncodeTiled(") + what + ") failed: " + std::to_string((int)r));
-    };
     if (!p.stride2) {
         cuuint64_t dims[3] = {(cuuint64_t)cin, (cuuint64_t)in.Wp, (cuuint64_t)in.N * in.Hp};
         cuuint64_t strides[2] = {(cuuint64_t)in.ldc * esz, (cuuint64_t)in.Wp * in.ldc * esz};
         cuuint32_t box[3] = {(cuuint32_t)p.BK, (cuuint32_t)p.TW, (cuuint32_t)p.TH};
-        cuuint32_t es[3] = {1, 1, 1};
-        check(enc(&plan.tmA, dtype, 3, in.base, dims, strides, box, es,
-                  CU_TENSOR_MAP_INTERLEAVE_NONE, swz, CU_TENSOR_MAP_L2_PROMOTION_L2_128B, CU_TENSOR_MAP_FLOAT_OOB_FILL_NONE), "A");
+        encode_tiled(&plan.tmA, dtype, 3, in.base, dims, strides, box, swz, CU_TENSOR_MAP_L2_PROMOTION_L2_128B, "A");
     } else {
         cuuint64_t dims[5] = {(cuuint64_t)cin, 2, (cuuint64_t)in.Wp / 2, 2, (cuuint64_t)in.N * in.Hp / 2};
         cuuint64_t strides[4] = {(cuuint64_t)in.ldc * esz, (cuuint64_t)in.ldc * 2 * esz, (cuuint64_t)in.Wp * in.ldc * esz,
                                  (cuuint64_t)in.Wp * in.ldc * 2 * esz};
         cuuint32_t box[5] = {(cuuint32_t)p.BK, 1, (cuuint32_t)p.TW, 1, (cuuint32_t)p.TH};
-        cuuint32_t es[5] = {1, 1, 1, 1, 1};
-        check(enc(&plan.tmA, dtype, 5, in.base, dims, strides, box, es,
-                  CU_TENSOR_MAP_INTERLEAVE_NONE, swz, CU_TENSOR_MAP_L2_PROMOTION_L2_128B, CU_TENSOR_MAP_FLOAT_OOB_FILL_NONE), "A");
+        encode_tiled(&plan.tmA, dtype, 5, in.base, dims, strides, box, swz, CU_TENSOR_MAP_L2_PROMOTION_L2_128B, "A");
     }
     {
         const cuuint64_t K = (cuuint64_t)p.size * p.size * cin;
         cuuint64_t dims[2] = {K, (cuuint64_t)c.ldn};
         cuuint64_t strides[1] = {K * esz};
         cuuint32_t box[2] = {(cuuint32_t)p.BK, (cuuint32_t)p.BN};
-        cuuint32_t es[2] = {1, 1};
-        check(enc(&plan.tmB, dtype, 2, const_cast<void *>(c.w), dims, strides, box, es,
-                  CU_TENSOR_MAP_INTERLEAVE_NONE, swz, CU_TENSOR_MAP_L2_PROMOTION_L2_256B, CU_TENSOR_MAP_FLOAT_OOB_FILL_NONE), "B");
+        encode_tiled(&plan.tmB, dtype, 2, const_cast<void *>(c.w), dims, strides, box, swz, CU_TENSOR_MAP_L2_PROMOTION_L2_256B, "B");
     }
     plan.tmO = plan.tmA; plan.tmO1 = plan.tmA; plan.tmR = plan.tmA;
     if (p.tma_epi && c.out.base) {
@@ -1509,10 +1603,8 @@
             cuuint64_t dims[3] = {(cuuint64_t)p.n, (cuuint64_t)t.Wp, (cuuint64_t)t.N * t.Hp};
             cuuint64_t strides[2] = {(cuuint64_t)t.ldc * oesz, (cuuint64_t)t.Wp * t.ldc * oesz};
             cuuint32_t box[3] = {(cuuint32_t)p.tma_epi, (cuuint32_t)std::min(p.TW, reg ? 64 : 128), (cuuint32_t)box_rows};
-            cuuint32_t es[3] = {1, 1, 1};
-            check(enc(tm, c.out_bf16 ? CU_TENSOR_MAP_DATA_TYPE_BFLOAT16 : CU_TENSOR_MAP_DATA_TYPE_FLOAT32, 3, t.base, dims, strides, box, es,
-                      CU_TENSOR_MAP_INTERLEAVE_NONE, p.tma_epi * oesz == 128 ? CU_TENSOR_MAP_SWIZZLE_128B : CU_TENSOR_MAP_SWIZZLE_64B,
-                      CU_TENSOR_MAP_L2_PROMOTION_L2_128B, CU_TENSOR_MAP_FLOAT_OOB_FILL_NONE), what);
+            encode_tiled(tm, c.out_bf16 ? CU_TENSOR_MAP_DATA_TYPE_BFLOAT16 : CU_TENSOR_MAP_DATA_TYPE_FLOAT32, 3, t.base, dims, strides, box,
+                         p.tma_epi * oesz == 128 ? CU_TENSOR_MAP_SWIZZLE_128B : CU_TENSOR_MAP_SWIZZLE_64B, CU_TENSOR_MAP_L2_PROMOTION_L2_128B, what);
         };
         const int box_rows = reg ? std::max(p.TH / 2, 1) : p.TH;
         encode_px(&plan.tmO, c.out, "output", box_rows);
@@ -1572,7 +1664,15 @@
     return plan;
 }
 
-struct StemPlan { StemTcP p; int grid; bool s2; };
+using StemS2Kernel = void (*)(CUtensorMap, StemTcP);
+struct StemPlan {
+    CUtensorMap tmO;
+    StemTcP p;
+    int grid;
+    bool s2;
+    StemS2Kernel k_f32, k_u8;
+    DevBuf<unsigned long long> stats;
+};
 int tc_stem_supported(const Layer &l, const TV &out) {
     return l.c == 3 && l.size == 3 && l.stride == 1 && l.pad == 1 && (l.n == 16 || l.n == 32) &&
            (l.activation == YB_LEAKY || l.activation == YB_LINEAR) && out.base && out.ldc % 8 == 0 &&
@@ -1595,7 +1695,7 @@
            out1.H == l0.h / 2 && out1.W == l0.w / 2 && out1.ldc % 8 == 0 && (reinterpret_cast<uintptr_t>(out1.base) & 15) == 0;
 }
 StemPlanPtr tc_stem_s2_make_plan(const Layer &l0, const Layer &l1, const TV &out1, const void *d_w, const float *d_bias,
-                                 const void *d_w1, const float *d_bias1, int max_grid) {
+                                 const void *d_w1, const float *d_bias1, const TcSwitches &sw) {
     StemPlanPtr sp(new StemPlan());
     sp->s2 = true;
     StemTcP &p = sp->p;
@@ -1607,24 +1707,38 @@
     const long ntiles = (long)p.N * p.xt * p.yt;
     if (ntiles >= INT_MAX) fatal_throw("stem plan: too many tiles");
     p.ntiles = (int)ntiles;
-    sp->grid = std::min(p.ntiles, grid_cap(2 * sm_count(), max_grid));
-    for (const void *f : {(const void *)k_stem_s2_tc<false>, (const void *)k_stem_s2_tc<true>}) {
-        if (cudaFuncSetAttribute(f, cudaFuncAttributeMaxDynamicSharedMemorySize, (int)S2_SMEM) != cudaSuccess ||
-            cudaFuncSetAttribute(f, cudaFuncAttributePreferredSharedMemoryCarveout, 100) != cudaSuccess)
+    sp->grid = std::min(p.ntiles, grid_cap(sm_count(), sw.grid));
+    {
+        cuuint64_t dims[4] = {64, (cuuint64_t)p.OW, (cuuint64_t)p.OH, (cuuint64_t)p.N};
+        const cuuint64_t px = (cuuint64_t)out1.ldc * 2;
+        cuuint64_t strides[3] = {px, px * out1.Wp, px * out1.Wp * out1.Hp};
+        cuuint32_t box[4] = {64, S2_TW, S2_TH, 1};
+        encode_tiled(&sp->tmO, CU_TENSOR_MAP_DATA_TYPE_BFLOAT16, 4, out1.base + (size_t)(out1.Wp + 1) * px, dims, strides, box,
+                     CU_TENSOR_MAP_SWIZZLE_128B, CU_TENSOR_MAP_L2_PROMOTION_L2_128B, "stem layer-1 output");
+    }
+    sp->k_f32 = sw.stats ? k_stem_s2_tc<false, true> : k_stem_s2_tc<false, false>;
+    sp->k_u8 = sw.stats ? k_stem_s2_tc<true, true> : k_stem_s2_tc<true, false>;
+    for (StemS2Kernel f : {sp->k_f32, sp->k_u8}) {
+        if (cudaFuncSetAttribute((const void *)f, cudaFuncAttributeMaxDynamicSharedMemorySize, (int)S2_SMEM) != cudaSuccess)
             fatal_throw("cudaFuncSetAttribute(k_stem_s2_tc) failed");
+    }
+    if (sw.stats) {
+        sp->stats.ensure(TC_NSTATS * (size_t)sp->grid);
+        p.stats = sp->stats.get();
+        cudaMemset(p.stats, 0, sizeof(unsigned long long) * TC_NSTATS * sp->grid);
     }
     return sp;
 }
 void tc_stem_launch(const StemPlan &sp, const float *d_in_nchw, cudaStream_t s) {
     StemTcP p = sp.p;
     p.in = d_in_nchw;
-    if (sp.s2) k_stem_s2_tc<false><<<sp.grid, 256, S2_SMEM, s>>>(p);
+    if (sp.s2) sp.k_f32<<<sp.grid, S2_THREADS, S2_SMEM, s>>>(sp.tmO, p);
     else k_stem_tc<false><<<sp.grid, 128, 0, s>>>(p);
 }
 void tc_stem_launch_u8(const StemPlan &sp, const unsigned char *d_in_hwc, cudaStream_t s) {
     StemTcP p = sp.p;
     p.in8 = d_in_hwc;
-    if (sp.s2) k_stem_s2_tc<true><<<sp.grid, 256, S2_SMEM, s>>>(p);
+    if (sp.s2) sp.k_u8<<<sp.grid, S2_THREADS, S2_SMEM, s>>>(sp.tmO, p);
     else k_stem_tc<true><<<sp.grid, 128, 0, s>>>(p);
 }
 
@@ -1661,13 +1775,20 @@
     cudaLaunchKernelEx(&cfg, P.kernel, P.tmA, P.tmB, P.tmO, P.tmO1, P.tmR, P.p);
 }
 
+namespace {
+void mean_stats(const unsigned long long *d_stats, int grid, double (&m)[TC_NSTATS]) {
+    std::vector<unsigned long long> h(TC_NSTATS * (size_t)grid);
+    cudaDeviceSynchronize();
+    cudaMemcpy(h.data(), d_stats, h.size() * sizeof(unsigned long long), cudaMemcpyDeviceToHost);
+    for (int k = 0; k < TC_NSTATS; ++k) m[k] = 0;
+    for (int b = 0; b < grid; ++b) for (int k = 0; k < TC_NSTATS; ++k) m[k] += (double)h[TC_NSTATS * b + k] / grid;
+}
+}
+
 void TcPlanDelete::operator()(TcPlan *plan) const {
     if (plan->p.stats) {
-        std::vector<unsigned long long> h(TC_NSTATS * (size_t)plan->grid);
-        cudaDeviceSynchronize();
-        cudaMemcpy(h.data(), plan->p.stats, h.size() * sizeof(unsigned long long), cudaMemcpyDeviceToHost);
-        double m[TC_NSTATS] = {0};
-        for (int b = 0; b < plan->grid; ++b) for (int k = 0; k < TC_NSTATS; ++k) m[k] += (double)h[TC_NSTATS * b + k] / plan->grid;
+        double m[TC_NSTATS];
+        mean_stats(plan->p.stats, plan->grid, m);
         fprintf(stderr, "TCSTATS %-28s tiles/cta %.1f kb %d sps %d BN %d | producer: wait_empty %.0f tma_issue %.0f total %.0f | ",
                 plan->desc, (double)plan->p.num_work / plan->grid, plan->p.kblocks, plan->p.sps, plan->p.BN,
                 m[STAT_PROD_WAIT_EMPTY], m[STAT_PROD_TMA_ISSUE], m[STAT_PROD_TOTAL]);
@@ -1679,6 +1800,15 @@
     }
     delete plan;
 }
-void TcPlanDelete::operator()(StemPlan *plan) const { delete plan; }
-
-}
+void TcPlanDelete::operator()(StemPlan *plan) const {
+    if (plan->p.stats) {
+        double m[TC_NSTATS];
+        mean_stats(plan->p.stats, plan->grid, m);
+        fprintf(stderr, "TCSTATS %-28s tiles/cta %.1f | stem: wait_empty %.0f total %.0f | layer 1: wait_full %.0f total %.0f | "
+                "store: wait_read %.0f\n", "stem + layer 1 (k_stem_s2_tc)", (double)plan->p.ntiles / plan->grid,
+                m[STAT_PROD_WAIT_EMPTY], m[STAT_PROD_TOTAL], m[STAT_CONS_WAIT_FULL], m[STAT_CONS_TOTAL], m[STAT_STORE_WAIT_READ]);
+    }
+    delete plan;
+}
+
+}
diff --git a/yolo2_light_b200/csrc/yb_conv_tc.cuh b/yolo2_light_b200/csrc/yb_conv_tc.cuh
--- a/yolo2_light_b200/csrc/yb_conv_tc.cuh
+++ b/yolo2_light_b200/csrc/yb_conv_tc.cuh
@@ -62,7 +62,7 @@
 StemPlanPtr tc_stem_make_plan(const Layer &l, const TV &out, const void *d_w_32x32_bf16, const float *d_bias);
 int tc_stem_s2_supported(const Layer &l0, const Layer &l1, const TV &out1);
 StemPlanPtr tc_stem_s2_make_plan(const Layer &l0, const Layer &l1, const TV &out1, const void *d_w_32x32_bf16,
-                                 const float *d_bias, const void *d_w1_bf16, const float *d_bias1, int max_grid);
+                                 const float *d_bias, const void *d_w1_bf16, const float *d_bias1, const TcSwitches &sw);
 void tc_stem_launch(const StemPlan &plan, const float *d_in_nchw, cudaStream_t s);
 void tc_stem_launch_u8(const StemPlan &plan, const unsigned char *d_in_hwc, cudaStream_t s);
 
diff --git a/yolo2_light_b200/csrc/yb_engine.cu b/yolo2_light_b200/csrc/yb_engine.cu
--- a/yolo2_light_b200/csrc/yb_engine.cu
+++ b/yolo2_light_b200/csrc/yb_engine.cu
@@ -662,7 +662,7 @@
         } else if (first == FIRST_STEM_TC || first == FIRST_STEM_S2) {
             const bool s2 = first == FIRST_STEM_S2;
             e.stem_plan = s2 ? tc_stem_s2_make_plan(l0, layer(1), e.out_tv[1], e.w_arena.get() + stem_w_off, bias(0),
-                                                    e.w_arena.get() + cw[1].w_bf16, bias(1), sw.tc.grid)
+                                                    e.w_arena.get() + cw[1].w_bf16, bias(1), sw.tc)
                              : tc_stem_make_plan(l0, e.out_tv[0], e.w_arena.get() + stem_w_off, bias(0));
             const StemPlan *sp = e.stem_plan.get();
             if (s2) ++e.n_tc;
```

After: 3225, median of 6. No clear change (+0.7%).
